# revdotcom/reverb

Measured on AMD Instinct MI355X. Metric: RTFx (audio-sec/wall-sec) Reverb-ASR attention_rescoring, higher is better.
Workload: dtype bf16

## Files before the change

### reverb_amd/_lib.py

```python
from __future__ import annotations

import ctypes as C
import os

_HERE = os.path.dirname(os.path.abspath(__file__))
LIB_PATH = os.path.join(_HERE, "librvb.so")

RVB_F32, RVB_BF16, RVB_FP8 = 0, 1, 2
ACT_NONE, ACT_SILU, ACT_RELU = 0, 1, 2
NORM_LN, NORM_AFFINE = 0, 1


class RvbError(RuntimeError):
    pass


class AudioInfo(C.Structure):
    _fields_ = [("container", C.c_int32), ("sample_format", C.c_int32), ("channels", C.c_int32), ("sample_rate", C.c_int32),
                ("bits_per_sample", C.c_int32), ("md5_checked", C.c_int32), ("frames", C.c_int64), ("decode_threads", C.c_int32),
                ("reserved", C.c_int32)]


class _SizedCfg(C.Structure):

# ... 104 lines not shown

class AttnTestArgs(C.Structure):
    _fields_ = ([(n, C.c_int32) for n in ("dtype", "heads", "dk", "nseq")] +
                [f for b in ("q", "k", "v", "out") for f in ((b, _f32p), (b[0] + "_rows", C.c_int32), (b[0] + "_stride", C.c_int32),
                                                             (b[0] + "_col", C.c_int32), ("pad_" + b, C.c_int32))] +
                [("p", _f32p), ("p_rows", C.c_int32), ("p_stride", C.c_int32), ("p_col", C.c_int32), ("p_off", C.c_int32),
                 ("bias_u", _f32p), ("bias_v", _f32p)] +
                [(n, _i32p) for n in ("q_start", "q_len", "kv_start", "kv_len", "q_pos0", "kv_index", "work")] +
                [(n, C.c_int32) for n in ("n_index", "n_work", "max_q", "q_block", "causal", "chunk", "left", "plain_order", "fold",
                                          "k_prefolded", "fold_kv_cap", "lab")] +
                [("ran", C.c_int32 * 8)])


class NormTestArgs(C.Structure):
    _fields_ = ([(n, C.c_int32) for n in ("dtype", "x_bf16", "mode", "silu", "out_f32", "out_fp8", "out2_fp8", "M", "d", "pad0")] +
                [(n, C.c_float) for n in ("eps", "eps2", "out_scale", "out2_scale")] +
                [(n, _f32p) for n in ("x", "gamma", "beta", "add", "gamma2", "beta2", "out", "out2")] +
                [("sat", C.c_uint32), ("sat2", C.c_uint32)])


_u32p = C.POINTER(C.c_uint32)

TEST_SIGNATURES = {
    "rvb_test_rownorm_ex": (C.c_int, [C.POINTER(NormTestArgs)]),
    "rvb_test_conv1_ex": (C.c_int, [C.c_int, _f32p, _f32p, _f32p, _f32p, _f32p, _f32p, C.c_int, C.c_int, C.c_int, C.c_int, C.c_float,
                                    _f32p, _u32p]),
    "rvb_test_embed": (C.c_int, [_f32p, C.c_int, _f32p, C.c_int, _i32p, _i32p, _f32p, C.c_int, C.c_int, C.c_float]),
    "rvb_test_amax_abs": (C.c_int, [C.c_int, _f32p, C.c_int64, _f32p]),
    "rvb_test_convert_f32": (C.c_int, [C.c_int, _f32p, _f32p, C.c_int64]),
    "rvb_test_gather_cache": (C.c_int, [C.c_void_p, C.c_void_p, _i32p, C.c_int, C.c_int, C.c_int, C.c_int]),
    "rvb_test_gather_pairs": (C.c_int, [_f32p, C.c_int, C.c_int64, _i32p, _i32p, C.c_int, _f32p]),
    "rvb_test_gemm": (C.c_int, [C.c_int, _f32p, _f32p, _f32p, _f32p, _f32p, C.c_int, C.c_int, C.c_int, C.c_float,
                                C.c_int, C.c_int, C.c_int, C.c_int, C.c_int, C.c_int, C.c_int]),
    "rvb_test_rownorm": (C.c_int, [C.c_int, _f32p, _f32p, _f32p, C.c_float, C.c_int, C.c_int, _f32p, _f32p, C.c_int,
                                   C.c_int, C.c_int]),
    "rvb_test_conv_block32": (C.c_int, [_f32p, _f32p, _f32p, _f32p, _f32p, _f32p, C.c_int, C.c_int, C.c_int]),
    "rvb_test_conv_s2sc": (C.c_int, [_f32p, _f32p, _f32p, _f32p, _f32p, _f32p, _f32p, C.c_int, C.c_int, C.c_int]),
    "rvb_test_conv1": (C.c_int, [C.c_int, _f32p, _f32p, _f32p, _f32p, _f32p, _f32p, C.c_int, C.c_int, C.c_int, C.c_int]),
    "rvb_test_conv_igemm_fp8": (C.c_int, [_f32p, _f32p, _f32p, _f32p, _f32p, _f32p, C.c_int, C.c_int, C.c_int, C.c_int, C.c_int, C.c_int, C.c_int,
                                           C.c_float, C.c_float, _f32p, _f32p, _f32p]),
    "rvb_test_joint_new": (C.c_void_p, [C.c_int, C.c_int, C.c_int, C.c_int, C.c_double, C.c_double, C.c_double]),
    "rvb_test_joint_free": (None, [C.c_void_p]),
    "rvb_test_joint_begin": (C.c_int, [C.c_void_p, C.c_int, _f32p, _i32p, C.c_int, C.c_float, C.c_float, _i32p, _i32p, _i32p, _i32p, _i32p,
                                       C.c_int]),
    "rvb_test_joint_finish": (C.c_int, [C.c_void_p, _f32p]),
    "rvb_test_joint_prefix": (C.c_int, [C.c_void_p, C.c_int, _i32p, _i32p]),
    "rvb_test_joint_result": (C.c_int, [C.c_void_p, _i32p, _i32p, _i32p, _f64p, _i32p, _f64p]),
    "rvb_test_glu_dwconv": (C.c_int, [C.c_int, _f32p, _f32p, _f32p, _f32p, _i32p, _f32p, C.c_int, C.c_int, C.c_int,
                                      C.c_int, C.c_int, _f32p, C.c_int]),
    "rvb_test_attention": (C.c_int, [C.c_int, _f32p, _f32p, _f32p, _f32p, _f32p, _f32p, _f32p, C.c_int, C.c_int,
                                     C.c_int, C.c_int, C.c_int, _i32p, _i32p, _i32p, _i32p, C.c_int, C.c_int]),
    "rvb_test_attention_trie": (C.c_int, [C.c_int, _f32p, _f32p, _f32p, _f32p, C.c_int, C.c_int, C.c_int, _i32p, _i32p, _i32p,
                                          _i32p, _i32p, _i32p, C.c_int, C.c_int, C.c_int]),
    "rvb_test_attention_ex": (C.c_int, [C.POINTER(AttnTestArgs)]),
    "rvb_test_attention_pos_bias": (C.c_int, [_f32p, C.c_int, C.c_int, C.c_int, C.c_int, _f32p, _f32p, C.c_int, C.c_int, C.c_float, _f32p]),
    "rvb_test_logsoftmax_topk": (C.c_int, [_f32p, C.c_int, C.c_int, C.c_int, C.c_float, C.c_int, _f32p, _i32p, _f32p]),
    "rvb_test_lse_gather": (C.c_int, [_f32p, C.c_int, C.c_int, _i32p, _f32p]),
    "rvb_test_ctc_viterbi": (C.c_int, [_f32p, C.c_int, C.c_int, _i32p, C.c_int, C.c_int, C.c_int, _i32p, _f32p]),
    "rvb_test_ctc_viterbi_wild": (C.c_int, [_f32p, C.c_int, C.c_int, _f32p, C.c_float, _i32p, C.c_int, C.c_int, C.c_int, _i32p, _f32p]),
    "rvb_test_ctc_viterbi_graph": (C.c_int, [_f32p, _i32p, C.c_int, C.c_int, _f32p, C.c_float, _i32p, _i32p, _i32p, _i32p, _u8p, C.c_int,
                                             C.c_int, _i32p, _i32p, _f32p]),
    "rvb_test_ctc_score": (C.c_int, [_f32p, C.c_int, C.c_int, _i32p, C.c_int, C.c_int, C.c_int, _f64p, _f32p, _f32p, _f32p, _i32p]),
    "rvb_test_ctc_score_batch": (C.c_int, [_f32p, _i32p, C.c_int, _i32p, _i32p, C.c_int, C.c_int, C.c_int, _f64p, _f32p, _f32p, _f32p,
                                           _i32p]),
    "rvb_test_ctc_find": (C.c_int, [_f32p, _i32p, C.c_int, C.c_int, _f32p, _i32p, _i32p, C.c_int, _f32p, C.c_int, C.c_int, C.c_int, C.c_int,
                                    _i64p, _i32p, _i32p, _f32p, _i32p, _i32p, _i32p, _f32p]),
    "rvb_test_gemm_glu": (C.c_int, [_f32p, _f32p, _f32p, _f32p, C.c_int, C.c_int, C.c_int]),
    "rvb_test_gemm_rowadd": (C.c_int, [_f32p, _f32p, _f32p, _f32p, _f32p, C.c_int, C.c_int, C.c_int, C.c_int, C.c_int, C.c_int]),
    "rvb_test_mp3_decode": (C.c_int64, [C.c_char_p, C.c_int64, C.c_int, _f32p, C.c_int64, _i64p, _i64p, C.c_int]),
    "rvb_test_mp3_hybrid": (C.c_int, [_f32p, _f32p, C.c_int, C.c_int, _f32p]),
    "rvb_test_mp3_polyphase": (C.c_int, [_f32p, _f32p, _i32p, _f32p]),
    "rvb_test_mp3_window": (C.c_int, [_f32p]),
    "rvb_test_mp3_huffman": (C.c_int, [C.c_int, C.POINTER(C.c_uint16), C.POINTER(C.c_uint8), _i32p]),
    "rvb_test_gemm_fp8": (C.c_int, [_f32p, _f32p, _f32p, _f32p, _f32p, C.c_int, C.c_int, C.c_int, C.c_float, C.c_float, C.c_int, C.c_int,
                                    C.c_float, _f32p, _f32p]),
    "rvb_test_rownorm_fp8": (C.c_int, [_f32p, _f32p, _f32p, C.c_float, C.c_int, C.c_int, C.c_int, C.c_float, _f32p, _f32p, _f32p,
                                       C.c_float, C.c_float, _f32p, _f32p]),
    "rvb_test_lse_gather_multi": (C.c_int, [_f32p, C.c_int, C.c_int, _i32p, _i32p, C.c_int, _f32p]),
    "rvb_test_row_xent": (C.c_int, [_f32p, C.c_int, C.c_int, C.c_int, _i32p, _i32p, _f32p, _f32p, _f64p, _i32p]),
    "rvb_test_host_pool": (C.c_int, [C.c_int, C.c_int, C.c_int]),
    "rvb_test_build_trie": (C.c_int, [_i32p, _i32p, _i32p, C.c_int, C.c_int, C.c_int, C.c_int, C.c_int, _i32p, _i32p, _i32p, _i32p, _i32p, _i32p,
                                      _i32p, _i32p, _i32p, _i32p, _i32p]),
    "rvb_test_fbank": (C.c_int, [_i16p, C.c_int64, _f32p]),
    "rvb_test_set_gemm_variant": (C.c_int, [C.c_int]),
    "rvb_test_set_gemm2_opts": (C.c_int, [C.c_int, C.c_int]),
    "rvb_test_gemm_timeline": (C.c_int, [C.c_int] * 6 + [C.POINTER(C.c_longlong), C.c_int, _i32p]),
    "rvb_test_gemm_bench": (C.c_int, [C.c_int, C.c_int, C.c_int, C.c_int, C.c_int, C.c_int, C.c_int, C.c_int, C.c_int,
                                      _f64p, _f64p]),
    "rvb_test_prefix_beam": (C.c_int, [_f32p, _i32p, C.c_int, C.c_int, C.c_int, _i32p, _i32p, _i32p, _i32p, _i32p,
                                       _f64p]),
    "rvb_test_prefix_beam_context": (C.c_int, [_f32p, _i32p, C.c_int, C.c_int, C.c_int, C.c_int, _i32p, _i32p, C.c_int, C.c_double,
                                               _i32p, _i32p, _i32p, _i32p, _i32p, _f64p, _f64p]),
    "rvb_test_context_walk": (C.c_int, [_i32p, _i32p, C.c_int, C.c_double, C.c_int, C.c_int, _i32p, C.c_int, _i32p, _f64p, _i32p,
                                        _f64p]),
    "rvb_test_window_stats": (C.c_int, [_f32p, C.c_int64, C.c_int64, C.c_int, C.c_int64, C.c_int, C.c_float, _f32p]),
    "rvb_test_sinc_conv": (C.c_int, [C.c_int, _f32p, C.c_int64, _f32p, C.c_int, C.c_int, C.c_int, C.c_int64, _f32p]),
    "rvb_test_pool_norm": (C.c_int, [C.c_int, C.c_int, _f32p, C.c_int, C.c_int, C.c_int, C.c_int, C.c_int, _f32p, _f32p, C.c_float,
                                     C.c_int, _f32p, C.c_int64, C.c_int64, C.c_int, _f32p, _f32p, C.c_float, C.c_float, _f32p]),
    "rvb_test_conv1d5": (C.c_int, [C.c_int, _f32p, C.c_int64, _f32p, _f32p, _f32p, C.c_int64]),
    "rvb_test_lstm_layer": (C.c_int, [C.c_int, _f32p, C.c_int, C.c_int, C.c_int, _f32p, _f32p, _f32p, _f32p, _f32p]),
    "rvb_test_classifier": (C.c_int, [C.c_int, _f32p, C.c_int, _f32p, _f32p, _f32p, C.POINTER(C.c_uint8), C.c_int64, C.c_int, C.c_int]),
    "rvb_test_tstp": (C.c_int, [C.c_int, _f32p, C.c_int, _i32p, _f32p, C.c_int, C.c_int, C.c_int, C.c_int, C.c_int, _f32p]),
    "rvb_test_conv2d": (C.c_int, [C.c_int, C.c_int, _f32p, _f32p, _f32p, _f32p, _f32p, C.c_int, C.c_int, C.c_int, C.c_int, C.c_int,
                                  C.c_int, C.c_int, C.c_int, _f32p, _f32p, C.c_int, C.c_int, C.c_int, C.c_int, _i32p]),
    "rvb_test_emb_stem": (C.c_int, [C.c_int, _f32p, C.c_int64, _i64p, C.c_int, C.c_int, C.c_int, C.c_int, C.c_int, C.c_int, _f32p, _f32p,
                                    _f32p, _f32p]),
}



class DiarCfg(_SizedCfg):
    _fields_ = [(n, C.c_int32) for n in (
        "struct_size", "dtype", "sample_rate", "window_samples", "step_samples", "sinc_filters", "sinc_channels", "lstm_hidden",
        "lstm_layers", "linear_dim", "linear_layers", "num_classes", "emb_channels", "emb_dim")]


DIAR_SIGNATURES = {
    "rvd_last_error": (C.c_char_p, []),
    "rvd_model_cfg_size": (C.c_int, []),
    "rvd_emb_windows_per_pass": (C.c_int, [_eng]),
    "rvd_create": (C.c_int, [C.POINTER(DiarCfg), C.c_int, C.POINTER(_eng)]),
    "rvd_destroy": (None, [_eng]),
    "rvd_load_tensor": (C.c_int, [_eng, C.c_char_p, _f32p, _i64p, C.c_int]),
    "rvd_finalize": (C.c_int, [_eng]),
    "rvd_num_windows": (C.c_int64, [_eng, C.c_int64]),
    "rvd_frames_per_window": (C.c_int, [_eng]),
    "rvd_upload_pcm": (C.c_int, [_eng, _i16p, C.c_int64]),
    "rvd_rerun_resident": (C.c_int, [_eng]),
    "rvd_resample_pcm": (C.c_int, [_eng, _i16p, C.c_int64, C.c_int, _i16p, _i64p]),
    "rvd_segment": (C.c_int, [_eng, C.c_int64, C.c_int, _f32p]),
    "rvd_get_classes": (C.c_int, [_eng, C.POINTER(C.c_uint8)]),
    "rvd_get_tap": (C.c_int, [_eng, C.c_char_p, _f32p]),
    "rvd_embed": (C.c_int, [_eng, _i64p, _f32p, C.c_int, _f32p]),
    "rvd_get_emb_fbank": (C.c_int, [_eng, C.c_int64, _f32p, _i32p]),
    "rvd_centroid_linkage": (C.c_int, [_eng, _f64p, C.c_int, C.c_int, _f64p]),
    "rvd_set_linkage_workgroups": (C.c_int, [_eng, C.c_int]),
    "rvd_get_emb_fp8": (C.c_int, [_eng, _i32p, _f32p, _i32p, C.POINTER(C.c_uint32)]),
    "rvd_set_emb_fp8_scales": (C.c_int, [_eng, _f32p, C.c_int32]),
    "rvd_set_profiling": (C.c_int, [_eng, C.c_int]),
    "rvd_reset_timings": (C.c_int, [_eng]),
    "rvd_get_timing": (C.c_int, [_eng, C.c_char_p, _f64p, _f64p, _i64p]),
}

_lib = None
_test_lib = None
TEST_LIB_PATH = os.path.join(_HERE, "librvb_test.so")


def load_test():
    global _test_lib
    if _test_lib is not None:
        return _test_lib
    if not os.path.exists(TEST_LIB_PATH):
        raise RvbError(f"{TEST_LIB_PATH} not found: run `python -m reverb_amd.build` (hipcc, gfx950)")
    lib = C.CDLL(TEST_LIB_PATH)
    for name, (res, args) in list(SIGNATURES.items()) + list(DIAR_SIGNATURES.items()) + list(TEST_SIGNATURES.items()):
        fn = getattr(lib, name)
        fn.restype = res
        fn.argtypes = args
    _test_lib = lib
    return lib


def load():
    global _lib
    if os.environ.get("RVB_LAB") == "1":
# ... 49 lines not shown
```

### reverb_amd/csrc/diar_engine.hip

```cpp
#include <cmath>
#include <cstdlib>
#include <cstring>
#include <map>
#include <string>
#include <vector>

#include "../../include/rvd.h"
#include "engine.h"

using namespace rvb;

#define RVD_TRY(expr) do { int _r = (expr); if (_r != OK) return _r; } while (0)

namespace {
struct LstmLayer { Linear ih; DevBuf whh; int in_pad = 0; };
constexpr int SINC_K = 251, SINC_STRIDE = 10, CONV_K = 5;
struct ConvW { DevBuf w, b, w_ig; int cin = 0, cout = 0, taps = 9, stride = 1;
               DevBuf w_ig_sc, b_sc;
               DevBuf w8, w8s; };
struct ResBlock { ConvW c1, c2, sc; bool has_sc = false; };
constexpr int FB_WIN = 400, FB_SHIFT = 160, FB_MEL = 80;
static int emb_batch() {
  static int v = [] { const char* e = getenv("RVD_EMB_BATCH"); const int x = e ? atoi(e) : 0; return x > 0 ? x : 768; }();
  return v;
}
#define EMB_BATCH (e->emb_batch > 0 ? e->emb_batch : (e->emb_batch = emb_batch()))
}

struct rvd_engine {
  rvd_model_cfg cfg;
  int device = 0, dtype = 0;
  int linkage_workgroups = 0;
  hipStream_t stream = nullptr;
  bool finalized = false;
  std::map<std::string, HostTensor> host;

  int f1 = 0, p1 = 0, f2 = 0, p2 = 0, f3 = 0, p3 = 0, cpad = 0;

  DevBuf filt, fsum;
  float wn_gamma = 1.f, wn_beta = 0.f;
  LNorm norm[3];
  Linear conv2, conv3;
  std::vector<LstmLayer> lstm;
  std::vector<Linear> lin;
  DevBuf cls_w, cls_b;
  DevBuf stage;

  DevBuf pcm, wave, craw;
  int64_t n_samples = 0, n_pad = 0, n_windows = 0, craw_frames = 0;

  DevBuf stats, a1, c2, a2, c3, a3, xproj, hA, hB, l0, l1, logp, cls;
  int last_W = 0;
  const void* last_lstm = nullptr;

  bool has_emb = false;
  DevBuf stem_w, stem_b;
  std::vector<std::vector<ResBlock>> stages;
  Linear seg1;
  DevBuf fb_window, fb_twiddle, fb_melw, fb_lo, fb_hi;
  DevBuf pcm_pad, emb_fb;
  int64_t emb_frames = 0;
  int nfr = 0;
  DevBuf act[4][4];
  int emb_batch = 0;
  bool emb_fp8 = false, want_fp8 = false;
  int emb_f8_state = 0;
  DevBuf act8[4][3], d_amax8, d_sat8;
  std::vector<float> scale8;
  int act_cap = 0;
  DevBuf e_win, e_mean, e_item_b, e_mask, e_stats, e_out;

  bool profiling = false;
  std::map<std::string, ProfEntry> prof;
  struct Pending { hipEvent_t a, b; std::string name; };
  std::vector<Pending> pending;
  std::vector<hipEvent_t> event_pool;
};

namespace {

struct DScope {
  rvd_engine* e; hipEvent_t a = nullptr, b = nullptr; std::string name;
  DScope(rvd_engine* e_, const char* n, double flops = 0.0) : e(e_), name(n) {
    auto& pe = e->prof[name];
    pe.launches += 1; pe.flops += flops;
    if (!e->profiling) return;
    auto get = [&]() { hipEvent_t ev; if (!e->event_pool.empty()) { ev = e->event_pool.back(); e->event_pool.pop_back(); } else (void)hipEventCreate(&ev); return ev; };
    a = get(); b = get();
    (void)hipEventRecord(a, e->stream);
  }
  ~DScope() { if (a) { (void)hipEventRecord(b, e->stream); e->pending.push_back({a, b, name}); } }
};
void drain(rvd_engine* e) {
  if (e->pending.empty()) return;
  (void)hipStreamSynchronize(e->stream);
  for (auto& p : e->pending) {
    float ms = 0.f;
    (void)hipEventElapsedTime(&ms, p.a, p.b);
    e->prof[p.name].ms += ms;
    e->event_pool.push_back(p.a); e->event_pool.push_back(p.b);
  }
  e->pending.clear();
}

int up_f32(rvd_engine* e, DevBuf& dst, const float* src, size_t n) {
  RVD_TRY(dst.ensure(n * 4));
  RVB_HIP_CHECK(hipMemcpyAsync(dst.p, src, n * 4, hipMemcpyHostToDevice, e->stream));
  RVB_HIP_CHECK(hipStreamSynchronize(e->stream));
  return OK;
}
int pack_T(rvd_engine* e, DevBuf& dst, const float* src, size_t n) {
  RVD_TRY(dst.ensure(n * dt_size(e->dtype)));
  if (e->dtype == DT_F32) return up_f32(e, dst, src, n);
  RVD_TRY(up_f32(e, e->stage, src, n));
  RVD_TRY(convert_f32(e->stream, e->dtype, e->stage.as<float>(), dst.p, n));
  RVB_HIP_CHECK(hipStreamSynchronize(e->stream));
  return OK;
}
int need(rvd_engine* e, const std::string& name, size_t numel, const HostTensor** out) {
  auto it = e->host.find(name);
  if (it == e->host.end()) { set_error("missing tensor: " + name); return E_STATE; }
  if (it->second.numel() != numel) {
    set_error("tensor " + name + " has " + std::to_string(it->second.numel()) + " elements, expected " + std::to_string(numel));
    return E_ARG;
  }
  *out = &it->second;
  return OK;
}
int pack_norm(rvd_engine* e, LNorm& n, const std::string& p, int d) {
  const HostTensor *g, *b;
  RVD_TRY(need(e, p + ".weight", d, &g));
  RVD_TRY(need(e, p + ".bias", d, &b));
  n.eps = 1e-5f;
  RVD_TRY(up_f32(e, n.g, g->data.data(), d));
  return up_f32(e, n.b, b->data.data(), d);
}

void sinc_filters(const float* low_hz_, const float* band_hz_, int npair, int sr, std::vector<float>* out, std::vector<float>* fsum) {
  const int K = SINC_K, half = K / 2;
  out->assign((size_t)2 * npair * K, 0.f);
  fsum->assign((size_t)2 * npair, 0.f);
  const double min_low = 50.0, min_band = 50.0;
// ... 137 lines not shown
  RVD_TRY(e->c2.ensure((size_t)R1 * CP * ts));
  RVD_TRY(e->a2.ensure((size_t)(R2 + 8) * CP * ts));
  RVD_TRY(e->c3.ensure((size_t)R2 * CP * ts));
  RVD_TRY(e->a3.ensure((size_t)R3 * CP * ts));
  RVD_TRY(e->xproj.ensure((size_t)R3 * 8 * H * ts));
  RVD_TRY(e->hA.ensure((size_t)R3 * 2 * H * ts));
  RVD_TRY(e->hB.ensure((size_t)R3 * 2 * H * ts));
  RVD_TRY(e->l0.ensure((size_t)R3 * c.linear_dim * ts));
  RVD_TRY(e->l1.ensure((size_t)R3 * c.linear_dim * ts));
  RVD_TRY(e->logp.ensure((size_t)R3 * c.num_classes * 4));
  RVD_TRY(e->cls.ensure((size_t)R3));

  { DScope sc(e, "window_stats");
    RVD_TRY(window_stats(e->stream, e->wave.as<float>(), first, W, c.step_samples, c.window_samples, 1e-5f, e->stats.as<float>())); }
  PoolNormArgs pn{};
  pn.W = W; pn.eps = 1e-5f;
  { DScope sc(e, "pool_norm");
    pn.x = nullptr; pn.frames_in = e->f1; pn.C = NF; pn.ld_out = NF;
    pn.gamma = e->norm[0].g.as<float>(); pn.beta = e->norm[0].b.as<float>(); pn.out = e->a1.p;
    pn.craw = e->craw.p; pn.craw_frame0 = first * (c.step_samples / SINC_STRIDE);
    pn.craw_frames_per_step = c.step_samples / SINC_STRIDE;
    pn.stats = e->stats.as<float>(); pn.fsum = e->fsum.as<float>(); pn.wn_gamma = e->wn_gamma; pn.wn_beta = e->wn_beta;
    RVD_TRY(pool_norm(e->stream, e->dtype, pn)); }
  RVD_TRY(run_sincnet_conv(e, e->a1.p, NF, e->conv2, e->c2.p, CP, R1));
  { DScope sc(e, "pool_norm");
    pn.x = e->c2.p; pn.rows_in = e->p1; pn.ld_in = CP; pn.frames_in = e->f2; pn.C = c.sinc_channels; pn.ld_out = CP;
    pn.gamma = e->norm[1].g.as<float>(); pn.beta = e->norm[1].b.as<float>(); pn.out = e->a2.p;
    RVD_TRY(pool_norm(e->stream, e->dtype, pn)); }
  RVD_TRY(run_sincnet_conv(e, e->a2.p, CP, e->conv3, e->c3.p, CP, R2));
  { DScope sc(e, "pool_norm");
    pn.x = e->c3.p; pn.rows_in = e->p2; pn.ld_in = CP; pn.frames_in = e->f3; pn.C = c.sinc_channels; pn.ld_out = CP;
    pn.gamma = e->norm[2].g.as<float>(); pn.beta = e->norm[2].b.as<float>(); pn.out = e->a3.p;
    RVD_TRY(pool_norm(e->stream, e->dtype, pn)); }

  const void* x = e->a3.p;
  int ldx = CP;
  for (int l = 0; l < c.lstm_layers; ++l) {
    RVD_TRY(run_gemm(e, "lstm_inproj", x, ldx, e->lstm[l].ih, e->xproj.p, 8 * H, R3, ACT_NONE));
    void* out = (l & 1) ? e->hB.p : e->hA.p;
    { DScope sc(e, "lstm_recurrence", 2.0 * (double)R3 * 8 * H * H);
      RVD_TRY(lstm_recurrence(e->stream, e->dtype, e->xproj.p, e->lstm[l].whh.p, out, W, e->p3)); }
    x = out; ldx = 2 * H;
  }
  e->last_lstm = x;
  for (int i = 0; i < c.linear_layers; ++i) {
    void* out = (i & 1) ? e->l1.p : e->l0.p;
    RVD_TRY(run_gemm(e, "linear", x, ldx, e->lin[i], out, c.linear_dim, R3, ACT_LRELU));
    x = out; ldx = c.linear_dim;
  }
  { DScope sc(e, "classifier");
    RVD_TRY(classifier_logsoftmax(e->stream, e->dtype, x, ldx, e->cls_w.as<float>(), e->cls_b.as<float>(), e->logp.as<float>(),
                                  e->cls.as<uint8_t>(), R3, ldx, c.num_classes)); }
  e->last_W = W;
  if (logp_out) {
    DScope sc(e, "d2h");
    RVB_HIP_CHECK(hipMemcpyAsync(logp_out, e->logp.p, (size_t)R3 * c.num_classes * 4, hipMemcpyDeviceToHost, e->stream));
  }
  RVB_HIP_CHECK(hipStreamSynchronize(e->stream));
  return OK;
}

int make_hamming_fbank_tables(rvd_engine* e) {
  const int NFFT = 512, NBIN = 257;
  const double PI = 3.14159265358979323846;
  std::vector<float> win(FB_WIN), tw(2 * 256), melw((size_t)FB_MEL * NBIN, 0.f);
  std::vector<int32_t> lo(FB_MEL, NBIN), hi(FB_MEL, 0);
  for (int i = 0; i < FB_WIN; ++i) win[i] = (float)(0.54 - 0.46 * std::cos(2.0 * PI * i / (FB_WIN - 1)));
  for (int k = 0; k < 256; ++k) { tw[2 * k] = (float)std::cos(2.0 * PI * k / NFFT); tw[2 * k + 1] = (float)(-std::sin(2.0 * PI * k / NFFT)); }
  auto mel = [](double f) { return 1127.0 * std::log(1.0 + f / 700.0); };
  const double mlo = mel(20.0), mhi = mel(8000.0), delta = (mhi - mlo) / (FB_MEL + 1);
  for (int m = 0; m < FB_MEL; ++m) {
    const double left = mlo + m * delta, center = left + delta, right = center + delta;
    for (int b = 0; b < NFFT / 2; ++b) {
      const double mf = mel(16000.0 / NFFT * b);
      const double w = std::max(0.0, std::min((mf - left) / (center - left), (right - mf) / (right - center)));
      if (w > 0.0) { melw[(size_t)m * NBIN + b] = (float)w; lo[m] = std::min(lo[m], b); hi[m] = std::max(hi[m], b + 1); }
    }
    if (hi[m] == 0) lo[m] = 0;
  }
  RVD_TRY(up_f32(e, e->fb_window, win.data(), win.size()));
  RVD_TRY(up_f32(e, e->fb_twiddle, tw.data(), tw.size()));
  RVD_TRY(up_f32(e, e->fb_melw, melw.data(), melw.size()));
  RVD_TRY(up_f32(e, e->fb_lo, (const float*)lo.data(), lo.size()));
  return up_f32(e, e->fb_hi, (const float*)hi.data(), hi.size());
}

int pack_conv_bn(rvd_engine* e, ConvW& c, const std::string& conv, const std::string& bn, int cout, int cin, int k, int stride) {
  const HostTensor *w, *g, *b, *m, *v;
  RVD_TRY(need(e, conv + ".weight", (size_t)cout * cin * k * k, &w));
  RVD_TRY(need(e, bn + ".weight", cout, &g));
  RVD_TRY(need(e, bn + ".bias", cout, &b));
  RVD_TRY(need(e, bn + ".running_mean", cout, &m));
  RVD_TRY(need(e, bn + ".running_var", cout, &v));
  const int CK = 64 / (int)dt_size(e->dtype);
  if (cin % CK) { set_error("embedding conv " + conv + ": input channels must be a multiple of " + std::to_string(CK)); return E_UNSUPPORTED; }
  const int taps = k * k;
  std::vector<float> pw((size_t)taps * cin * cout), pb(cout), sc(cout);
  for (int o = 0; o < cout; ++o) {
    sc[o] = g->data[o] / std::sqrt(v->data[o] + 1e-5f);
    pb[o] = b->data[o] - m->data[o] * sc[o];
  }
  conv_pack_direct(w->data.data(), sc.data(), cout, cin, taps, CK, pw.data());
  c.cin = cin; c.cout = cout; c.taps = taps; c.stride = stride;
  RVD_TRY(pack_T(e, c.w, pw.data(), pw.size()));
  if (conv_igemm_packed(e->dtype, k, stride, cin, cout)) {
    std::vector<float> pg((size_t)cout * taps * cin);
    conv_pack_igemm(w->data.data(), sc.data(), cout, cin, taps, (size_t)taps * cin, pg.data());
    RVD_TRY(pack_T(e, c.w_ig, pg.data(), pg.size()));
    if (e->emb_fp8 && cin % 128 == 0) {
      std::vector<uint8_t> q(pg.size());
      std::vector<float> ws(cout);
      const size_t K = (size_t)taps * cin;
      for (int o = 0; o < cout; ++o) {
        float am = 0.f;
        for (size_t kk = 0; kk < K; ++kk) am = std::max(am, std::fabs(pg[(size_t)o * K + kk]));
        ws[o] = am > 0.f ? am / 448.f : 1.f;
        const float inv = 1.f / ws[o];
        for (size_t kk = 0; kk < K; ++kk) q[(size_t)o * K + kk] = f32_to_fp8_host(pg[(size_t)o * K + kk] * inv);
      }
      RVD_TRY(c.w8.ensure(q.size()));
      RVB_HIP_CHECK(hipMemcpyAsync(c.w8.p, q.data(), q.size(), hipMemcpyHostToDevice, e->stream));
      RVD_TRY(up_f32(e, c.w8s, ws.data(), ws.size()));
      RVB_HIP_CHECK(hipStreamSynchronize(e->stream));
    }
  }
  return up_f32(e, c.b, pb.data(), pb.size());
}

int pack_fused_shortcut(rvd_engine* e, ResBlock& B, const std::string& p) {
  const char* f = lab_env("RVD_CONV_SC_FUSE");
  if ((f && atoi(f) == 0) || !B.has_sc || !B.c2.w_ig.p || B.sc.cin % 64 || B.sc.taps != 1) return OK;
  const int cout = B.c2.cout, cin = B.c2.cin, c2 = B.sc.cin;
  const HostTensor *w, *g, *b, *m, *v, *ws, *gs, *bs, *ms, *vs;
  RVD_TRY(need(e, p + ".conv2.weight", (size_t)cout * cin * 9, &w));
  RVD_TRY(need(e, p + ".bn2.weight", cout, &g));
  RVD_TRY(need(e, p + ".bn2.bias", cout, &b));
  RVD_TRY(need(e, p + ".bn2.running_mean", cout, &m));
  RVD_TRY(need(e, p + ".bn2.running_var", cout, &v));
  RVD_TRY(need(e, p + ".shortcut.0.weight", (size_t)cout * c2, &ws));
  RVD_TRY(need(e, p + ".shortcut.1.weight", cout, &gs));
  RVD_TRY(need(e, p + ".shortcut.1.bias", cout, &bs));
  RVD_TRY(need(e, p + ".shortcut.1.running_mean", cout, &ms));
  RVD_TRY(need(e, p + ".shortcut.1.running_var", cout, &vs));
  std::vector<float> pg((size_t)cout * (9 * (size_t)cin + c2)), pb(cout), sc(cout), ss(cout);
  for (int o = 0; o < cout; ++o) {
    sc[o] = g->data[o] / std::sqrt(v->data[o] + 1e-5f);
    ss[o] = gs->data[o] / std::sqrt(vs->data[o] + 1e-5f);
    pb[o] = (b->data[o] - m->data[o] * sc[o]) + (bs->data[o] - ms->data[o] * ss[o]);
  }
  conv_pack_fused_shortcut(w->data.data(), sc.data(), ws->data.data(), ss.data(), cout, cin, c2, pg.data());
  RVD_TRY(pack_T(e, B.c2.w_ig_sc, pg.data(), pg.size()));
  return up_f32(e, B.c2.b_sc, pb.data(), pb.size());
}

int finalize_embedding(rvd_engine* e) {
  const rvd_model_cfg& c = e->cfg;
  const std::string S = "embedding.resnet.";
  const int m = c.emb_channels;
  if (m != 32) { set_error("embedding: this build supports m_channels = 32 (ResNet34 of pyannote/wespeaker-voxceleb-resnet34-LM)"); return E_UNSUPPORTED; }
  { const char* f8 = lab_env("RVD_EMB_FP8"); e->emb_fp8 = (e->want_fp8 || (f8 && atoi(f8) == 1)) && e->dtype == DT_BF16; e->emb_f8_state = 0; }
  const HostTensor *w, *g, *b, *mu, *v;
  RVD_TRY(need(e, S + "conv1.weight", (size_t)m * 9, &w));
  RVD_TRY(need(e, S + "bn1.weight", m, &g));
  RVD_TRY(need(e, S + "bn1.bias", m, &b));
  RVD_TRY(need(e, S + "bn1.running_mean", m, &mu));
  RVD_TRY(need(e, S + "bn1.running_var", m, &v));
  std::vector<float> sw((size_t)m * 9), sb(m);
// ... 261 lines not shown
      g.A = e->e_stats.p; g.W = e->seg1.w.p; g.bias = e->seg1.b.as<float>(); g.C = e->e_out.p;
      g.M = ni; g.N = c.emb_dim; g.K = stats; g.lda = stats; g.ldw = stats; g.ldc = c.emb_dim; g.alpha = 1.f; g.act = ACT_NONE;
      g.out_f32 = 1;
      RVD_TRY(gemm(e->stream, e->dtype, g)); }
    RVB_HIP_CHECK(hipMemcpyAsync(emb_out + (size_t)i0 * c.emb_dim, e->e_out.p, (size_t)ni * c.emb_dim * 4, hipMemcpyDeviceToHost, e->stream));
    RVB_HIP_CHECK(hipStreamSynchronize(e->stream));
    i0 = i1;
  }
  return OK;
}

int fetch_T(rvd_engine* e, const void* src, int64_t rows, int ld, int cols, float* out) {
  const size_t ts = dt_size(e->dtype);
  std::vector<char> tmp((size_t)rows * ld * ts);
  RVB_HIP_CHECK(hipMemcpy(tmp.data(), src, tmp.size(), hipMemcpyDeviceToHost));
  for (int64_t r = 0; r < rows; ++r)
    for (int cc = 0; cc < cols; ++cc)
      out[r * cols + cc] = e->dtype == DT_BF16 ? bf16_to_f32(((const bf16_t*)tmp.data())[r * ld + cc]) : ((const float*)tmp.data())[r * ld + cc];
  return OK;
}

}

extern "C" {

const char* rvd_last_error(void) { return rvb::last_error(); }

int rvd_model_cfg_size(void) { return (int)sizeof(rvd_model_cfg); }

int rvd_emb_windows_per_pass(rvd_engine* e) {
  if (!e) { set_error("rvd_emb_windows_per_pass: null engine"); return E_ARG; }
  return EMB_BATCH;
}

int rvd_create(const rvd_model_cfg* cfg, int device, rvd_engine** out) {
  if (!cfg || !out) { set_error("rvd_create: null argument"); return E_ARG; }
  *out = nullptr;
  if (cfg->struct_size != (int32_t)sizeof(rvd_model_cfg)) {
    set_error("rvd_create: ABI mismatch: rvd_model_cfg.struct_size is " + std::to_string(cfg->struct_size) + ", this library's struct has " +
              std::to_string(sizeof(rvd_model_cfg)) + " bytes (bind it field by field from include/rvd.h)");
    return E_ARG;
  }
  if (cfg->dtype != DT_F32 && cfg->dtype != DT_BF16 && cfg->dtype != RVB_FP8) { set_error("rvd_create: dtype must be RVB_F32, RVB_BF16 or RVB_FP8"); return E_ARG; }
  if (cfg->lstm_hidden != 128 || cfg->sinc_filters != 80 || cfg->sinc_filters % 8 || cfg->sinc_channels < 1 || cfg->sinc_channels > 64 ||
      cfg->lstm_layers < 1 || cfg->linear_layers < 0 || cfg->linear_layers > 2 || (cfg->linear_layers && cfg->linear_dim % 8) ||
      cfg->linear_dim > 256 || cfg->num_classes < 1 || cfg->num_classes > 16 || cfg->sample_rate != 16000 ||
      cfg->step_samples % (SINC_STRIDE * 4) || cfg->step_samples <= 0 || cfg->window_samples < 4000) {
    set_error("rvd_create: unsupported model dimensions (this build: 80 sinc filters, <= 64 conv channels, LSTM hidden 128, 16 kHz)");
    return E_ARG;
  }
  int ndev = 0;
  if (hipGetDeviceCount(&ndev) != hipSuccess || ndev <= device || device < 0) {
    set_error("rvd_create: no HIP device " + std::to_string(device) + " (this library has no CPU fallback)");
    return E_HIP;
  }
  RVB_HIP_CHECK(hipSetDevice(device));
  rvd_engine* e = new rvd_engine();
  e->cfg = *cfg; e->device = device;
  e->want_fp8 = cfg->dtype == RVB_FP8;
  e->dtype = e->want_fp8 ? (int)DT_BF16 : cfg->dtype;
  e->cfg.dtype = e->dtype;
  RVB_HIP_CHECK(hipStreamCreateWithFlags(&e->stream, hipStreamNonBlocking));
  e->f1 = (cfg->window_samples - SINC_K) / SINC_STRIDE + 1; e->p1 = e->f1 / 3;
  e->f2 = e->p1 - (CONV_K - 1); e->p2 = e->f2 / 3;
  e->f3 = e->p2 - (CONV_K - 1); e->p3 = e->f3 / 3;
  e->cpad = 64;
  *out = e;
  return OK;
}

void rvd_destroy(rvd_engine* e) {
  if (!e) return;
  (void)hipSetDevice(e->device);
  (void)hipStreamSynchronize(e->stream);
  drain(e);
  for (auto ev : e->event_pool) (void)hipEventDestroy(ev);
  DevBuf* bufs[] = {&e->filt, &e->fsum, &e->cls_w, &e->cls_b, &e->stage, &e->pcm, &e->wave, &e->craw, &e->stats, &e->a1, &e->c2,
                    &e->a2, &e->c3, &e->a3, &e->xproj, &e->hA, &e->hB, &e->l0, &e->l1, &e->logp, &e->cls, &e->conv2.w, &e->conv2.b,
                    &e->conv3.w, &e->conv3.b};
  for (auto* b : bufs) b->release();
  for (auto& n : e->norm) { n.g.release(); n.b.release(); }
  for (auto& l : e->lstm) { l.ih.w.release(); l.ih.b.release(); l.whh.release(); }
  for (auto& l : e->lin) { l.w.release(); l.b.release(); }
  DevBuf* ebufs[] = {&e->stem_w, &e->stem_b, &e->seg1.w, &e->seg1.b, &e->fb_window, &e->fb_twiddle, &e->fb_melw, &e->fb_lo, &e->fb_hi,
                     &e->pcm_pad, &e->emb_fb, &e->e_win, &e->e_mean, &e->e_item_b, &e->e_mask, &e->e_stats, &e->e_out};
  for (auto* b : ebufs) b->release();
  for (auto& st : e->stages)
    for (auto& blk : st)
      for (ConvW* cw : {&blk.c1, &blk.c2, &blk.sc}) { cw->w.release(); cw->b.release(); cw->w_ig.release(); cw->w_ig_sc.release(); cw->b_sc.release(); cw->w8.release(); cw->w8s.release(); }
  for (auto& row : e->act) for (auto& b : row) b.release();
  (void)hipStreamDestroy(e->stream);
  delete e;
}

int rvd_load_tensor(rvd_engine* e, const char* name, const float* host, const int64_t* shape, int ndim) {
  if (!e || !name || !host || ndim < 0 || (ndim && !shape)) { set_error("rvd_load_tensor: null argument"); return E_ARG; }
  if (e->finalized) { set_error("rvd_load_tensor: engine already finalized"); return E_STATE; }
  HostTensor t;
  t.shape.assign(shape, shape + ndim);
  t.data.assign(host, host + t.numel());
  e->host[name] = std::move(t);
  return OK;
}

int rvd_finalize(rvd_engine* e) {
  if (!e) { set_error("rvd_finalize: null engine"); return E_ARG; }
  if (e->finalized) { set_error("rvd_finalize: already finalized"); return E_STATE; }
  RVB_HIP_CHECK(hipSetDevice(e->device));
  return finalize_impl(e);
}

int64_t rvd_num_windows(const rvd_engine* e, int64_t n) {
  if (!e || n <= 0) return 0;
  const int64_t win = e->cfg.window_samples, step = e->cfg.step_samples;
  const int64_t full = n >= win ? (n - win) / step + 1 : 0;
  const bool tail = n < win || (n - win) % step > 0;
  return full + (tail ? 1 : 0);
}
int rvd_frames_per_window(const rvd_engine* e) { return e ? e->p3 : 0; }

static int prepare_audio(rvd_engine* e, int64_t n);

int rvd_upload_pcm(rvd_engine* e, const int16_t* pcm, int64_t n) {
  if (!e || !pcm || n <= 0) { set_error("rvd_upload_pcm: null or empty audio"); return E_ARG; }
  if (!e->finalized) { set_error("rvd_upload_pcm: finalize the model first"); return E_STATE; }
  RVB_HIP_CHECK(hipSetDevice(e->device));
  RVD_TRY(e->pcm.ensure((size_t)n * 2));
  { DScope sc(e, "h2d");
    RVB_HIP_CHECK(hipMemcpyAsync(e->pcm.p, pcm, (size_t)n * 2, hipMemcpyHostToDevice, e->stream)); }
  return prepare_audio(e, n);
}

int rvd_rerun_resident(rvd_engine* e) {
  if (!e) { set_error("rvd_rerun_resident: null engine"); return E_ARG; }
  if (e->n_samples <= 0 || !e->pcm.p) { set_error("rvd_rerun_resident: upload audio first"); return E_STATE; }
  RVB_HIP_CHECK(hipSetDevice(e->device));
  return prepare_audio(e, e->n_samples);
}

int rvd_resample_pcm(rvd_engine* e, const int16_t* pcm, int64_t n, int sample_rate, int16_t* out, int64_t* n_out) {
  if (!e || !pcm || n <= 0 || !n_out) { set_error("rvd_resample_pcm: null or empty audio"); return E_ARG; }
  if (sample_rate < 1000 || sample_rate > 384000) { set_error("rvd_resample_pcm: sample rate out of range"); return E_ARG; }
  const int target = e->cfg.sample_rate;
  std::vector<float> ker;
  int orig, nw, width, K;
  resample_taps(sample_rate, target, &ker, &orig, &nw, &width, &K);
  const int64_t m = ((int64_t)nw * n + orig - 1) / orig;
  if (!out) { *n_out = m; return OK; }
  if (*n_out < m) { set_error("rvd_resample_pcm: output buffer too small"); return E_ARG; }
  *n_out = m;
  RVB_HIP_CHECK(hipSetDevice(e->device));
  DevBuf src, taps, res, dst;
  int r = src.ensure((size_t)n * 2 + 16);
  if (r == OK) r = taps.ensure(ker.size() * 4);
  if (r == OK) r = res.ensure((size_t)m * 4);
  if (r == OK) r = dst.ensure((size_t)m * 2);
  if (r == OK && hipMemcpyAsync(src.p, pcm, (size_t)n * 2, hipMemcpyHostToDevice, e->stream) != hipSuccess) r = E_HIP;
  if (r == OK && hipMemcpyAsync(taps.p, ker.data(), ker.size() * 4, hipMemcpyHostToDevice, e->stream) != hipSuccess) r = E_HIP;
  if (r == OK) { DScope sc(e, "resample"); r = resample(e->stream, src.as<int16_t>(), n, taps.as<float>(), orig, nw, width, K, res.as<float>(), m); }
  if (r == OK) r = round_to_i16(e->stream, res.as<float>(), m, dst.as<int16_t>());
  if (r == OK && hipMemcpyAsync(out, dst.p, (size_t)m * 2, hipMemcpyDeviceToHost, e->stream) != hipSuccess) r = E_HIP;
  if (hipStreamSynchronize(e->stream) != hipSuccess && r == OK) r = E_HIP;
  src.release(); taps.release(); res.release(); dst.release();
  if (r == E_HIP) set_error("rvd_resample_pcm: device copy or kernel failed");
  return r;
}

static int prepare_audio(rvd_engine* e, int64_t n) {
  const rvd_model_cfg& c = e->cfg;
  e->n_samples = n;
  e->n_windows = rvd_num_windows(e, n);
  e->n_pad = (e->n_windows - 1) * c.step_samples + c.window_samples;
  e->craw_frames = (e->n_pad - SINC_K) / SINC_STRIDE + 1;
  RVD_TRY(e->wave.ensure((size_t)e->n_pad * 4));
  RVD_TRY(e->craw.ensure((size_t)e->craw_frames * c.sinc_filters * dt_size(e->dtype)));
  { DScope sc(e, "pcm_to_float");
    RVD_TRY(pcm_to_float(e->stream, e->pcm.as<int16_t>(), n, e->wave.as<float>(), e->n_pad)); }
  { DScope sc(e, "sinc_conv", 2.0 * (double)e->craw_frames * c.sinc_filters * SINC_K);
    RVD_TRY(sinc_conv(e->stream, e->dtype, e->wave.as<float>(), e->filt.as<float>(), e->craw.p, e->craw_frames, c.sinc_filters,
                      SINC_K, SINC_STRIDE)); }
  if (e->has_emb) {
    e->emb_frames = (e->n_pad - FB_WIN) / FB_SHIFT + 1;
    RVD_TRY(e->pcm_pad.ensure((size_t)e->n_pad * 2));
    RVD_TRY(e->emb_fb.ensure((size_t)e->emb_frames * FB_MEL * 4));
    RVB_HIP_CHECK(hipMemsetAsync(e->pcm_pad.p, 0, (size_t)e->n_pad * 2, e->stream));
    RVB_HIP_CHECK(hipMemcpyAsync(e->pcm_pad.p, e->pcm.p, (size_t)n * 2, hipMemcpyDeviceToDevice, e->stream));
    DScope sc(e, "emb_fbank");
    FbankTables t{e->fb_window.as<float>(), e->fb_twiddle.as<float>(), e->fb_melw.as<float>(), e->fb_lo.as<int>(), e->fb_hi.as<int>()};
    RVD_TRY(fbank(e->stream, e->pcm_pad.as<int16_t>(), e->emb_frames, e->emb_fb.as<float>(), t));
    RVD_TRY(e->e_mean.ensure((size_t)e->n_windows * FB_MEL * 4));
    RVD_TRY(emb_window_mean(e->stream, e->emb_fb.as<float>(), nullptr, (int)e->n_windows, c.step_samples / FB_SHIFT, e->nfr, e->e_mean.as<float>()));
  }
  RVB_HIP_CHECK(hipStreamSynchronize(e->stream));
  return OK;
}

int rvd_segment(rvd_engine* e, int64_t first_window, int n_windows, float* logp_out) {
  if (!e) { set_error("rvd_segment: null engine"); return E_ARG; }
  RVB_HIP_CHECK(hipSetDevice(e->device));
  return segment_impl(e, first_window, n_windows, logp_out);
}

int rvd_get_classes(rvd_engine* e, uint8_t* out) {
  if (!e || !out) { set_error("rvd_get_classes: null argument"); return E_ARG; }
  if (e->last_W <= 0) { set_error("rvd_get_classes: no rvd_segment call yet"); return E_STATE; }
  RVB_HIP_CHECK(hipSetDevice(e->device));
  RVB_HIP_CHECK(hipMemcpy(out, e->cls.p, (size_t)e->last_W * e->p3, hipMemcpyDeviceToHost));
  return OK;
}

int rvd_get_tap(rvd_engine* e, const char* name, float* out) {
  if (!e || !name || !out) { set_error("rvd_get_tap: null argument"); return E_ARG; }
  if (e->last_W <= 0) { set_error("rvd_get_tap: no rvd_segment call yet"); return E_STATE; }
  RVB_HIP_CHECK(hipSetDevice(e->device));
  const int64_t R3 = (int64_t)e->last_W * e->p3;
  if (!strcmp(name, "sincnet")) return fetch_T(e, e->a3.p, R3, e->cpad, e->cfg.sinc_channels, out);
  if (!strcmp(name, "lstm")) return fetch_T(e, e->last_lstm, R3, 2 * e->cfg.lstm_hidden, 2 * e->cfg.lstm_hidden, out);
  set_error(std::string("rvd_get_tap: unknown tap ") + name);
  return E_ARG;
}

int rvd_embed(rvd_engine* e, const int64_t* win, const float* mask, int n, float* emb_out) {
  if (!e || !win || !mask || !emb_out || n < 0) { set_error("rvd_embed: null argument"); return E_ARG; }
  RVB_HIP_CHECK(hipSetDevice(e->device));
  return embed_impl(e, win, mask, n, emb_out);
}
int rvd_get_emb_fbank(rvd_engine* e, int64_t window, float* out, int32_t* n_frames) {
  if (!e || !out) { set_error("rvd_get_emb_fbank: null argument"); return E_ARG; }
  if (!e->has_emb || e->n_windows == 0) { set_error("rvd_get_emb_fbank: needs an embedding model and uploaded audio"); return E_STATE; }
  if (window < 0 || window >= e->n_windows) { set_error("rvd_get_emb_fbank: window outside the uploaded audio"); return E_ARG; }
  RVB_HIP_CHECK(hipSetDevice(e->device));
  const int64_t f0 = window * (e->cfg.step_samples / FB_SHIFT);
  RVB_HIP_CHECK(hipMemcpy(out, e->emb_fb.as<float>() + f0 * FB_MEL, (size_t)e->nfr * FB_MEL * 4, hipMemcpyDeviceToHost));
  if (n_frames) *n_frames = e->nfr;
  return OK;
}

int rvd_centroid_linkage(rvd_engine* e, const double* X, int n, int d, double* Z) {
  if (!e || !X || !Z || n < 1 || d < 1) { set_error("rvd_centroid_linkage: bad argument"); return E_ARG; }
  if (n > 46000) { set_error("rvd_centroid_linkage: more than 46000 points"); return E_UNSUPPORTED; }
  if (n == 1) return OK;
  RVB_HIP_CHECK(hipSetDevice(e->device));
  DevBuf dX, dD, dI, dM, dZ, dC;
  int rc = OK;
  do {
    if ((rc = dC.ensure(4096)) != OK) break;
    if ((rc = dX.ensure((size_t)n * d * 8)) != OK) break;
    if ((rc = dD.ensure((size_t)n * n * 8)) != OK) break;
    if ((rc = dI.ensure((size_t)3 * n * 4)) != OK) break;
    if ((rc = dM.ensure((size_t)n * 8)) != OK) break;
    if ((rc = dZ.ensure((size_t)(n - 1) * 4 * 8)) != OK) break;
    std::vector<int> init((size_t)3 * n);
    for (int i = 0; i < n; ++i) { init[i] = i; init[n + i] = -1; ((uint16_t*)&init[2 * (size_t)n])[i] = 1; }
    std::vector<double> inf(n, INFINITY);
    (void)hipMemcpyAsync(dX.p, X, (size_t)n * d * 8, hipMemcpyHostToDevice, e->stream);
    (void)hipMemcpyAsync(dI.p, init.data(), init.size() * 4, hipMemcpyHostToDevice, e->stream);
    (void)hipMemcpyAsync(dM.p, inf.data(), (size_t)n * 8, hipMemcpyHostToDevice, e->stream);
    (void)hipStreamSynchronize(e->stream);
    {
      DScope sc(e, "linkage");
      rc = centroid_linkage(e->stream, dX.as<double>(), n, d, dD.as<double>(), (uint16_t*)(dI.as<int>() + 2 * n), dI.as<int>(),
                            dI.as<int>() + n, dM.as<double>(), dZ.as<double>(), dC.p, e->linkage_workgroups);
    }
    if (rc != OK) break;
    if (hipMemcpyAsync(Z, dZ.p, (size_t)(n - 1) * 4 * 8, hipMemcpyDeviceToHost, e->stream) != hipSuccess ||
        hipStreamSynchronize(e->stream) != hipSuccess) {
      set_error(std::string("rvd_centroid_linkage: ") + hipGetErrorString(hipGetLastError()));
      rc = E_HIP;
      break;
    }
    { double retries = 0.0;
// ... 74 lines not shown
```

### reverb_amd/csrc/engine.h

```cpp
#pragma once
#include <condition_variable>
#include <functional>
#include <map>
#include <memory>
#include <mutex>
#include <string>
#include <thread>
#include <vector>

#include "../../include/rvb.h"
#include "kernels.h"
#include "search.h"

namespace rvb {

struct HostTensor {
  std::vector<float> data;
  std::vector<int64_t> shape;
  size_t numel() const { size_t n = 1; for (auto s : shape) n *= (size_t)s; return n; }
};

struct DevBuf {
  void* p = nullptr;
  size_t bytes = 0;
// ... 120 lines not shown
           int V, int blank_id, bool allow_wild = false);
  int begin(hipStream_t s);
  bool touches(int r0, int nrows) const;
  int advance(hipStream_t s, const float* lp, int ld, int r0, int nrows, const float* wmax = nullptr, float bias = 0.f);
  int finish(hipStream_t s, int32_t* states , float* score );
  void release();
};

struct CtcGraphAligner {
  std::vector<GraphSeq> seq;
  std::vector<int32_t> h_tokens, h_arc_off, h_finals, h_rows;
  std::vector<uint32_t> h_arcs;
  int max_N = 0, blank = 0;
  bool has_wild = false;
  size_t alpha_floats = 0, bp_bytes = 0;
  int64_t total_frames = 0;
  DevBuf d_tokens, d_arc_off, d_arcs, d_finals, d_rows, d_seqs, d_alpha, d_bp, d_states, d_score;
  int plan(const char* who, const int32_t* node_tokens, const int32_t* n_nodes, const int32_t* pred_off, const int32_t* preds,
           const uint8_t* is_final, int n_seq, const std::vector<std::vector<int32_t>>& seq_rows, int V, int blank_id);
  int begin(hipStream_t s);
  bool touches(int r0, int nrows) const;
  int advance(hipStream_t s, const float* lp, int ld, int r0, int nrows, const float* wmax = nullptr, float bias = 0.f);
  int finish(hipStream_t s, int32_t* states , float* score );
  void release();
};

struct CtcScorer {
  CtcAligner lat;
  bool post = false;
  DevBuf d_csum, d_loglik, d_llhat, d_coff, d_arows, d_beta, d_z, d_acc;
  int plan(const char* who, const int32_t* tokens, const int32_t* tok_lens, int n_seq, const std::vector<std::vector<int32_t>>& seq_rows,
           int V, int blank_id);
  int begin(hipStream_t s, bool posteriors);
  int advance(hipStream_t s, const float* lp, int ld, int r0, int nrows);
  int finish_forward(hipStream_t s, double* loglik );
  int advance_backward(hipStream_t s, const float* lp, int ld, int r0, int nrows);
  int finish_backward(hipStream_t s, float* occupancy, float* mean_frame, float* peak_post, int32_t* peak_frame );
  void release();
};


struct CtcFinder {
  std::vector<FindSeq> seq;
  std::vector<FindPhrase> phr;
  std::vector<int32_t> h_tokens, h_rows;
  int blank = 0, max_cand = 0;
  DevBuf d_tokens, d_rows, d_seqs, d_phr, d_h, d_st, d_count, d_cend, d_cstart, d_cscore;
  int plan(const char* who, const int32_t* tokens, const int32_t* tok_lens, int n_phrases, const float* threshold,
           const std::vector<std::vector<int32_t>>& seq_rows, int V, int blank_id, int max_candidates);
  int begin(hipStream_t s);
  bool touches(int r0, int nrows) const;
  int advance(hipStream_t s, const float* lp, int ld, int r0, int nrows, const float* wmax);
  int finish(hipStream_t s, int max_hits, int32_t* n_hits, int32_t* start, int32_t* end, float* score, int64_t* n_candidates,
             int32_t* raw_end = nullptr, int32_t* raw_start = nullptr, float* raw_score = nullptr);
  void release();
};

}

struct rvb_engine {
  rvb_model_cfg cfg;
  int device = 0;
  int dtype = 0;
  bool fp8 = false;
  int f8_state = 0;
  std::vector<rvb::F8Scales> f8;
  std::vector<unsigned> f8_groups;
  rvb::DevBuf d_amax;
  bool f8_conv2 = false;
  float f8_x1 = 0.f;
  rvb::DevBuf d_f8sat;
  hipStream_t stream = nullptr;
  bool finalized = false;

  std::map<std::string, rvb::HostTensor> host;

  rvb::DevBuf cmvn_mean, cmvn_istd, conv1_w, conv1_b;
  rvb::Linear conv2, embed_out, ctc;
  rvb::LNorm enc_after;
  std::vector<rvb::EncLayer> enc;
  rvb::Decoder dec_l, dec_r;
  rvb::DevBuf pe_f32;
  int pe_rows = 0;
  rvb::DevBuf fb_window, fb_twiddle, fb_melw, fb_lo, fb_hi;
  rvb::DevBuf stage;

  rvb::DevBuf pcm, feats;
  rvb::DevBuf pcm_next;
  hipStream_t copy_stream = nullptr;
  hipEvent_t pcm_ready = nullptr, pcm_free = nullptr;
  bool pcm_pending = false;
  int64_t n_samples_next = 0;
  rvb::DevBuf wave_f32, rs_kernel;
  rvb::DevBuf wave_in;
  bool pcm_is_float = false;
  int dec_chunk = 0, dec_left = -1;
  int64_t n_samples = 0, n_frames = 0, feat_rows = 0;

  int B = 0, T0 = 0, T1 = 0, F1 = 0, T2 = 0, F2 = 0, beam = 0;
  std::vector<int32_t> in_lens, enc_lens;
  rvb::DevBuf d_feats_in, X1, X2, x, xn, y, h, ao, dconv, enc_out, logits, topv, topi;
  rvb::DevBuf d_enc_lens, d_seq_start, d_seq_len, d_aux_i32;
  float* h_topv = nullptr;
  int32_t* h_topi = nullptr;
  size_t h_top_cap = 0;
  struct Slice { int c0, nb; hipEvent_t ev; bool done; };
  std::vector<Slice> slices;
  std::vector<hipEvent_t> slice_event_pool;
  int xattn_max_rows = 0;
  const int* cur_lens = nullptr;
  std::vector<rvb::PrefixResult> nbest;
  std::shared_ptr<const rvb::ContextGraph> context_graph;
  std::vector<rvb::RescoreResult> rescored;
  std::vector<rvb::TrieBatch> trie_l;
  rvb::HostPool pool;
  std::vector<rvb::JointResult> joint;
  std::vector<rvb::DevBuf> jkv;
  rvb::DevBuf jlogp, jpair_row, jpair_tok, jpair_out;
  int64_t joint_rows = 0, joint_steps = 0;
  float last_blank_penalty = 0.f;
  std::vector<std::vector<int>> attn_tokens;
  std::vector<float> attn_scores;
  rvb::DevBuf atopv, atopi;
  std::vector<rvb::DevBuf> kcache, vcache, kcache2, vcache2, memkv;
  rvb::DevBuf dx, dxn, dy, dh, dqkv, dq, dao, kvmem, d_tok, d_pos, d_tgt, d_logp;
  rvb::DevBuf d_hq_start, d_hq_len, d_hkv_start, d_hkv_len;
  rvb::DevBuf d_hq_pos0, d_hpath_start, d_hpath_len, d_path, d_work, d_tgt_ptr;
  int64_t rescore_rows = 0, rescore_pairs = 0;
  rvb::DevBuf d_xlse, d_xsum, d_xtop;

  struct StreamState {
    bool active = false;
    int offset = 0;
    int cache_len = 0;
    std::vector<rvb::DevBuf> kv, kv2;
    int cnn_rows = 0;
    std::vector<rvb::DevBuf> cnn, cnn2;
  } stream_st;
  rvb::DevBuf d_stream_i32;

  rvb::CtcAligner aligner;
  rvb::CtcScorer scorer;
  rvb::CtcFinder finder;
  rvb::CtcGraphAligner graph_aligner;
  rvb::DevBuf align_lp, align_tv, align_ti, align_row, align_col, align_out;

  void* comm = nullptr;
  int comm_world = 1, comm_rank = 0;
  rvb::DevBuf comm_send, comm_recv;

  int profiling = 0;
  std::map<std::string, rvb::ProfEntry> prof;
  struct Pending { hipEvent_t a, b; std::string name; };
  std::vector<Pending> pending;
  std::vector<hipEvent_t> event_pool;
};
```

### reverb_amd/csrc/engine.hip

```cpp
#include "engine.h"

#include <algorithm>
#include <atomic>
#include <condition_variable>
#include <functional>
#include <mutex>
#include <chrono>
#include <cmath>
#include <cstdlib>
#include <cstring>
#include <thread>

namespace rvb {

static thread_local std::string g_err;
void set_error(const std::string& msg) { g_err = msg; }
const char* last_error() { return g_err.c_str(); }

int DevBuf::ensure(size_t n) {
  if (n <= bytes && p) return OK;
  if (p) { (void)hipFree(p); p = nullptr; bytes = 0; }
  if (n == 0) n = 16;
  hipError_t err = hipMalloc(&p, n);
  if (err != hipSuccess) {
    p = nullptr;
    (void)hipGetLastError();
    set_error("hipMalloc of " + std::to_string(n) + " bytes failed: " + hipGetErrorString(err));
    return E_NOMEM;
  }
  bytes = n;
  return OK;
}
void DevBuf::release() { if (p) (void)hipFree(p); p = nullptr; bytes = 0; }

#define RVB_TRY(expr) do { int _r = (expr); if (_r != OK) return _r; } while (0)

struct Scope {
  rvb_engine* e; hipEvent_t a = nullptr, b = nullptr; std::string name;
  Scope(rvb_engine* e_, const char* n, double flops = 0.0, double bytes = 0.0) : e(e_), name(n) {
    auto& pe = e->prof[name];
    pe.launches += 1; pe.flops += flops; pe.bytes += bytes;
    if (e->profiling == 0 || (e->profiling == 2 && name != "gemm" && name != "gemm_fp8")) return;
    auto get = [&]() { hipEvent_t ev; if (!e->event_pool.empty()) { ev = e->event_pool.back(); e->event_pool.pop_back(); } else (void)hipEventCreate(&ev); return ev; };
    a = get(); b = get();
    (void)hipEventRecord(a, e->stream);
  }
  ~Scope() {
    if (!a) return;
    (void)hipEventRecord(b, e->stream);
    e->pending.push_back({a, b, name});
  }
};
static void drain_prof(rvb_engine* e) {
  if (e->pending.empty()) return;
  (void)hipStreamSynchronize(e->stream);
  for (auto& p : e->pending) {
    float ms = 0.f;
    (void)hipEventElapsedTime(&ms, p.a, p.b);
    e->prof[p.name].ms += ms;
    e->event_pool.push_back(p.a); e->event_pool.push_back(p.b);
  }
  e->pending.clear();
}

static int upload_f32(rvb_engine* e, DevBuf& dst, const float* src, size_t n) {
  RVB_TRY(dst.ensure(n * 4));
  RVB_HIP_CHECK(hipMemcpyAsync(dst.p, src, n * 4, hipMemcpyHostToDevice, e->stream));
  return OK;
}
static int upload_i32(rvb_engine* e, DevBuf& dst, const int32_t* src, size_t n) {
  RVB_TRY(dst.ensure(n * 4 + 16));
  if (n) RVB_HIP_CHECK(hipMemcpyAsync(dst.p, src, n * 4, hipMemcpyHostToDevice, e->stream));
  return OK;
}
static int pack_T(rvb_engine* e, DevBuf& dst, const float* src, size_t n) {
  RVB_TRY(dst.ensure(n * dt_size(e->dtype)));
  if (e->dtype == DT_F32) {
    RVB_HIP_CHECK(hipMemcpyAsync(dst.p, src, n * 4, hipMemcpyHostToDevice, e->stream));
    return OK;
  }
  RVB_TRY(e->stage.ensure(n * 4));
  RVB_HIP_CHECK(hipMemcpyAsync(e->stage.p, src, n * 4, hipMemcpyHostToDevice, e->stream));
  return convert_f32(e->stream, e->dtype, e->stage.as<float>(), dst.p, n);
// ... 44 lines not shown
}
static int pack_norm(rvb_engine* e, LNorm& n, const std::string& p, int d, float eps) {
  const HostTensor *g, *b;
  RVB_TRY(need(e, p + ".weight", d, &g));
  RVB_TRY(need(e, p + ".bias", d, &b));
  n.eps = eps;
  RVB_TRY(upload_f32(e, n.g, g->data.data(), d));
  return upload_f32(e, n.b, b->data.data(), d);
}
static int pack_concat(rvb_engine* e, Linear& L, const std::vector<std::string>& names, int out_each, int in, bool f8 = false) {
  std::vector<float> w((size_t)names.size() * out_each * in), b((size_t)names.size() * out_each);
  for (size_t i = 0; i < names.size(); ++i) {
    const HostTensor *tw, *tb;
    RVB_TRY(need(e, names[i] + ".weight", (size_t)out_each * in, &tw));
    RVB_TRY(need(e, names[i] + ".bias", out_each, &tb));
    memcpy(w.data() + i * (size_t)out_each * in, tw->data.data(), (size_t)out_each * in * 4);
    memcpy(b.data() + i * (size_t)out_each, tb->data.data(), (size_t)out_each * 4);
  }
  int r = pack_linear(e, L, w.data(), b.data(), (int)names.size() * out_each, in, f8);
  if (r == OK) (void)hipStreamSynchronize(e->stream);
  return r;
}
static int pack_lsl(rvb_engine* e, Linear& L, const std::string& p, int d, const float* cat, int ncat) {
  std::vector<float> w((size_t)d * d, 0.f), b(d, 0.f);
  for (int i = 0; i < ncat; ++i) {
    const HostTensor *tw, *tb;
    const std::string n = p + ".language_layers." + std::to_string(i);
    RVB_TRY(need(e, n + ".weight", (size_t)d * d, &tw));
    RVB_TRY(need(e, n + ".bias", d, &tb));
    const float c = cat[i];
    if (i == 0) {
      for (size_t k = 0; k < w.size(); ++k) w[k] = c * tw->data[k];
      for (int k = 0; k < d; ++k) b[k] = c * tb->data[k];
    } else {
      for (size_t k = 0; k < w.size(); ++k) w[k] = w[k] + c * tw->data[k];
      for (int k = 0; k < d; ++k) b[k] = b[k] + c * tb->data[k];
    }
  }
  int r = pack_linear(e, L, w.data(), b.data(), d, d);
  if (r == OK) (void)hipStreamSynchronize(e->stream);
  return r;
}

static void make_pe(int rows, int d, std::vector<float>* pe) {
  pe->assign((size_t)rows * d, 0.f);
  const float c = (float)(-(std::log(10000.0) / (double)d));
  for (int i = 0; i < d; i += 2) {
    const float div = std::exp((float)i * c);
    for (int pos = 0; pos < rows; ++pos) {
      const float ang = (float)pos * div;
      (*pe)[(size_t)pos * d + i] = std::sin(ang);
      if (i + 1 < d) (*pe)[(size_t)pos * d + i + 1] = std::cos(ang);
    }
  }
}

static int make_fbank_tables(rvb_engine* e) {
  const int WIN = 400, NFFT = 512, NBIN = 257, NMEL = 80;
  const double PI = 3.14159265358979323846;
  std::vector<float> win(WIN), tw(2 * 256), melw((size_t)NMEL * NBIN, 0.f);
  std::vector<int32_t> lo(NMEL, NBIN), hi(NMEL, 0);
  for (int i = 0; i < WIN; ++i) win[i] = (float)std::pow(0.5 - 0.5 * std::cos(2.0 * PI * i / (WIN - 1)), 0.85);
  for (int k = 0; k < 256; ++k) { tw[2 * k] = (float)std::cos(2.0 * PI * k / NFFT); tw[2 * k + 1] = (float)(-std::sin(2.0 * PI * k / NFFT)); }
  auto mel = [](double f) { return 1127.0 * std::log(1.0 + f / 700.0); };
  const double mlo = mel(20.0), mhi = mel(8000.0), delta = (mhi - mlo) / (NMEL + 1);
  for (int m = 0; m < NMEL; ++m) {
    const double left = mlo + m * delta, center = left + delta, right = center + delta;
    for (int b = 0; b < NFFT / 2; ++b) {
      const double mf = mel(16000.0 / NFFT * b);
      const double up = (mf - left) / (center - left), down = (right - mf) / (right - center);
      const double w = std::max(0.0, std::min(up, down));
      if (w > 0.0) {
        melw[(size_t)m * NBIN + b] = (float)w;
        lo[m] = std::min(lo[m], b); hi[m] = std::max(hi[m], b + 1);
      }
    }
    if (hi[m] == 0) lo[m] = 0;
  }
  RVB_TRY(upload_f32(e, e->fb_window, win.data(), win.size()));
  RVB_TRY(upload_f32(e, e->fb_twiddle, tw.data(), tw.size()));
  RVB_TRY(upload_f32(e, e->fb_melw, melw.data(), melw.size()));
  RVB_TRY(upload_i32(e, e->fb_lo, lo.data(), lo.size()));
  RVB_TRY(upload_i32(e, e->fb_hi, hi.data(), hi.size()));
  RVB_HIP_CHECK(hipStreamSynchronize(e->stream));
  return OK;
}

static int out_frames(int T0) { const int T1 = (T0 - 3) / 2 + 1; return (T1 - 3) / 2 + 1; }

static const AttnArgs& with_lab(AttnArgs& a) { attention_lab_switches(a); return a; }

static int reset_f8sat(rvb_engine* e) {
  static const int on = lab_env("RVB_FP8_SAT") ? atoi(lab_env("RVB_FP8_SAT")) : 1;
  if (!on) return OK;
  RVB_TRY(e->d_f8sat.ensure((e->enc.size() + 1) * 8 * 4));
  RVB_HIP_CHECK(hipMemsetAsync(e->d_f8sat.p, 0, (e->enc.size() + 1) * 8 * 4, e->stream));
  return OK;
}

static double gemm_alg_bytes(const rvb_engine* e, const GemmArgs& g) {
  const double es = g.in_fp8 ? 1.0 : (double)dt_size(e->dtype);
  const double a = g.conv ? (double)(g.M / (g.cT2 * g.cF2)) * g.cT1 * g.cF1 * g.cC * es : (double)g.M * g.K * es;
  const double c = (double)g.M * (g.act == ACT_GLU ? g.N / 2 : g.N) * (g.out_fp8 ? 1.0 : (g.out_f32 ? 4.0 : (double)dt_size(e->dtype)));
  return a + (double)g.N * g.K * es + (g.bias ? 4.0 * g.N : 0.0) + c + (g.res ? 4.0 * (double)g.M * g.N : 0.0);
}

static constexpr int GLU_FUSE_DEFAULT = 1;
static int run_gemm(rvb_engine* e, const void* A, int lda, const Linear& L, void* C, int ldc, int M, bool out_f32,
                    float alpha = 1.f, int act = ACT_NONE, const float* res = nullptr, int ldres = 0) {
  GemmArgs g;
  memset(&g, 0, sizeof(g));
  g.A = A; g.W = L.w.p; g.bias = L.b.as<float>(); g.res = res; g.C = C;
  g.M = M; g.N = L.out; g.K = L.in; g.lda = lda; g.ldw = L.in; g.ldc = ldc; g.ldres = ldres;
  g.alpha = alpha; g.act = act; g.out_f32 = out_f32 ? 1 : 0;
  Scope sc(e, "gemm", 2.0 * M * (double)L.out * L.in, gemm_alg_bytes(e, g));
  return gemm(e->stream, e->dtype, g);
}
static int run_norm(rvb_engine* e, const float* x, const LNorm& n, void* out, bool out_f32, int M, int d,
                    int mode = NORM_LN, int silu = 0, const void* add = nullptr, const LNorm* second = nullptr,
                    void* out2 = nullptr, float out8 = 0.f, float out2_8 = 0.f, bool x_bf16 = false, unsigned* sat = nullptr,
                    unsigned* sat2 = nullptr) {
  NormArgs a;
  a.sat = sat; a.sat2 = sat2;
  a.x_bf16 = x_bf16 ? 1 : 0;
  a.x = x; a.gamma = n.g.as<float>(); a.beta = n.b.as<float>(); a.eps = n.eps; a.mode = mode; a.silu = silu;
  a.add = add; a.out = out; a.out_f32 = out_f32 ? 1 : 0; a.M = M; a.d = d;
  if (second) { a.gamma2 = second->g.as<float>(); a.beta2 = second->b.as<float>(); a.eps2 = second->eps; a.out2 = out2; }
  if (out8 > 0.f) { a.out_fp8 = 1; a.out_inv_scale = 1.f / out8; }
  if (out2_8 > 0.f) { a.out2_fp8 = 1; a.out2_inv_scale = 1.f / out2_8; }
  Scope sc(e, "rownorm");
  return rownorm(e->stream, e->dtype, a);
}
static int run_gemm8(rvb_engine* e, const void* A8, int lda, const Linear& L, void* C, int ldc, int M, float a_scale, int out_kind,
                     float out_scale = 1.f, float alpha = 1.f, int act = ACT_NONE, const float* res = nullptr, int ldres = 0,
                     unsigned* sat = nullptr) {
  GemmArgs g;
  memset(&g, 0, sizeof(g));
  g.sat = sat;
  g.A = A8; g.W = L.w8.p; g.bias = L.b.as<float>(); g.res = res; g.C = C;
  g.M = M; g.N = L.out; g.K = L.in; g.lda = lda; g.ldw = L.in; g.ldc = ldc; g.ldres = ldres;
  g.alpha = alpha; g.act = act; g.out_f32 = out_kind == 1; g.out_fp8 = out_kind == 2; g.in_fp8 = 1;
  g.a_scale = a_scale; g.w_scale = L.wscale.as<float>(); g.out_inv_scale = 1.f / out_scale;
  if (!L.w8.p) { set_error("fp8 GEMM on a layer without fp8 weights"); return E_STATE; }
  Scope sc(e, "gemm_fp8", 2.0 * M * (double)L.out * L.in, gemm_alg_bytes(e, g));
  return gemm(e->stream, e->dtype, g);
}

static int pack_decoder(rvb_engine* e, Decoder& D, const std::string& p, int nblocks, const float* cat, int ncat) {
  const int d = e->cfg.d_model, V = e->cfg.vocab, ff = e->cfg.dec_ffn_dim;
  D.present = false;
  if (nblocks <= 0 || !find(e, p + ".embed.0.weight")) return OK;
  const HostTensor* emb;
  RVB_TRY(need(e, p + ".embed.0.weight", (size_t)V * d, &emb));
  RVB_TRY(upload_f32(e, D.embed, emb->data.data(), emb->data.size()));
  RVB_TRY(pack_norm(e, D.after, p + ".after_norm", d, 1e-5f));
  RVB_TRY(pack_named_linear(e, D.out, p + ".output_layer", V, d));
  D.layers.resize(nblocks);
  for (int j = 0; j < nblocks; ++j) {
    DecLayer& L = D.layers[j];
    const std::string q = p + ".decoders." + std::to_string(j);
    L.is_lsl = find(e, q + ".language_layers.0.weight") != nullptr;
    const float eps = L.is_lsl ? 1e-12f : 1e-5f;
    RVB_TRY(pack_concat(e, L.self_qkv, {q + ".self_attn.linear_q", q + ".self_attn.linear_k", q + ".self_attn.linear_v"}, d, d));
    RVB_TRY(pack_named_linear(e, L.self_out, q + ".self_attn.linear_out", d, d));
    RVB_TRY(pack_named_linear(e, L.src_q, q + ".src_attn.linear_q", d, d));
    RVB_TRY(pack_concat(e, L.src_kv, {q + ".src_attn.linear_k", q + ".src_attn.linear_v"}, d, d));
// ... 747 lines not shown
      t->path.push_back(node);
      asks.push_back({node, j < h.len ? seq(h, j) : eos});
    }
    const int n_own = t->R - first_new;
    t->hq_start.push_back(first_new); t->hq_len.push_back(n_own); t->hq_pos0.push_back(n_own ? own_pos0 : 0);
    t->hkv_len.push_back(h.len + 1);
    for (int q0 = 0; q0 < n_own; q0 += 16) { t->work.push_back((int32_t)t->hq_start.size() - 1); t->work.push_back(q0); }
  }
  if (cur_chunk >= 0) t->crow_len[cur_chunk] = t->R - t->crow_start[cur_chunk];
  for (int b = 0; b < B; ++b) t->max_chunk_rows = std::max(t->max_chunk_rows, t->crow_len[b]);
  t->P = (int)asks.size();
  t->tgt_ptr.assign(t->R + 1, 0);
  for (auto& a : asks) t->tgt_ptr[a.first + 1]++;
  for (int r = 0; r < t->R; ++r) t->tgt_ptr[r + 1] += t->tgt_ptr[r];
  std::vector<int32_t> fill(t->tgt_ptr.begin(), t->tgt_ptr.end() - 1);
  t->tgt.assign(t->P, 0); t->pair_slot.assign(t->P, 0);
  for (int p = 0; p < t->P; ++p) { const int slot = fill[asks[p].first]++; t->tgt[slot] = asks[p].second; t->pair_slot[p] = slot; }
}

static void build_chunk_trie(rvb_engine* e, int b, bool reversed, int sos, int eos, TrieBatch* t) {
  const PrefixResult& pr = e->nbest[b];
  std::vector<HypRef> hyps(pr.nbest.size());
  for (size_t i = 0; i < hyps.size(); ++i) hyps[i] = {b, (int)i, (int)pr.nbest[i].size(), 0};
  if (reversed)
    build_trie_range(hyps.data(), hyps.data() + hyps.size(), b, 1, sos, eos,
                     [&](const HypRef& h, int j) { return pr.nbest[h.idx][h.len - 1 - j]; }, t);
  else
    build_trie_range(hyps.data(), hyps.data() + hyps.size(), b, 1, sos, eos, [&](const HypRef& h, int j) { return pr.nbest[h.idx][j]; }, t);
}

static void merge_tries(const std::vector<TrieBatch>& part, TrieBatch* t) {
  const int B = (int)part.size();
  *t = TrieBatch();
  size_t nR = 0, nH = 0, nPath = 0, nP = 0, nW = 0;
  for (const TrieBatch& c : part) { nR += c.R; nH += c.hq_start.size(); nPath += c.path.size(); nP += c.P; nW += c.work.size(); }
  t->tok.reserve(nR); t->pos.reserve(nR); t->path.reserve(nPath); t->work.reserve(nW);
  t->hq_start.reserve(nH); t->hq_len.reserve(nH); t->hq_pos0.reserve(nH); t->hkv_start.reserve(nH); t->hkv_len.reserve(nH);
  t->tgt.reserve(nP); t->pair_slot.reserve(nP); t->tgt_ptr.reserve(nR + 1);
  t->crow_start.assign(B, 0); t->crow_len.assign(B, 0);
  for (int b = 0; b < B; ++b) {
    const TrieBatch& c = part[b];
    const int32_t R0 = t->R, H0 = (int32_t)t->hq_start.size(), PATH0 = (int32_t)t->path.size(), P0 = t->P;
    t->crow_start[b] = c.R ? R0 : 0; t->crow_len[b] = c.R;
    t->max_chunk_rows = std::max(t->max_chunk_rows, c.R);
    t->tok.insert(t->tok.end(), c.tok.begin(), c.tok.end());
    t->pos.insert(t->pos.end(), c.pos.begin(), c.pos.end());
    for (int32_t v : c.path) t->path.push_back(v + R0);
    for (int32_t v : c.hq_start) t->hq_start.push_back(v + R0);
    t->hq_len.insert(t->hq_len.end(), c.hq_len.begin(), c.hq_len.end());
    t->hq_pos0.insert(t->hq_pos0.end(), c.hq_pos0.begin(), c.hq_pos0.end());
    for (int32_t v : c.hkv_start) t->hkv_start.push_back(v + PATH0);
    t->hkv_len.insert(t->hkv_len.end(), c.hkv_len.begin(), c.hkv_len.end());
    for (size_t k = 0; k + 1 < c.work.size(); k += 2) { t->work.push_back(c.work[k] + H0); t->work.push_back(c.work[k + 1]); }
    for (int r = 0; r < c.R; ++r) t->tgt_ptr.push_back(c.tgt_ptr[r] + P0);
    t->tgt.insert(t->tgt.end(), c.tgt.begin(), c.tgt.end());
    for (int32_t v : c.pair_slot) t->pair_slot.push_back(v + P0);
    t->R += c.R; t->P += c.P;
  }
  t->tgt_ptr.push_back(t->P);
}

static void build_trie_parallel(rvb_engine* e, bool reversed, TrieBatch* t) {
  const int B = e->B, sos = e->cfg.sos_id, eos = e->cfg.eos_id;
  std::vector<TrieBatch> part(B);
  std::atomic<int> next(0);
  auto work = [&]() {
    for (int b = next.fetch_add(1); b < B; b = next.fetch_add(1)) build_chunk_trie(e, b, reversed, sos, eos, &part[b]);
  };
  e->pool.run(std::max(1u, std::min<unsigned>(search_threads(), (unsigned)B / 4)), work);
  merge_tries(part, t);
}

static int decoder_memory_kv(rvb_engine* e, Decoder& D, int M) {
  const int d = e->cfg.d_model;
  const size_t es = dt_size(e->dtype);
  for (auto& L : D.layers) {
    RVB_TRY(L.kvmem.ensure((size_t)M * 2 * d * es));
    RVB_TRY(run_gemm(e, e->enc_out.p, d, L.src_kv, L.kvmem.p, 2 * d, M, false));
  }
  D.kv_ready = true;
  return OK;
}

struct XentRows { std::vector<float> lse; std::vector<double> sum_x; std::vector<int32_t> top1; };
static int decoder_forward(rvb_engine* e, Decoder& D, const TrieBatch& t, std::vector<float>* logp, XentRows* xent = nullptr) {
  const rvb_model_cfg& c = e->cfg;
  const int d = c.d_model, heads = c.dec_heads, dk = d / heads, ff = c.dec_ffn_dim, V = c.vocab;
  const int M = e->B * e->T2, R = t.R, nhyp = (int)t.hq_start.size();
  const size_t es = dt_size(e->dtype);
  RVB_TRY(upload_i32(e, e->d_tok, t.tok.data(), R));
  RVB_TRY(upload_i32(e, e->d_pos, t.pos.data(), R));
  RVB_TRY(upload_i32(e, e->d_tgt, t.tgt.data(), t.P));
  RVB_TRY(upload_i32(e, e->d_tgt_ptr, t.tgt_ptr.data(), R + 1));
  RVB_TRY(upload_i32(e, e->d_path, t.path.data(), t.path.size()));
  RVB_TRY(upload_i32(e, e->d_work, t.work.data(), t.work.size()));
  RVB_TRY(upload_i32(e, e->d_hq_start, t.hq_start.data(), nhyp));
  RVB_TRY(upload_i32(e, e->d_hq_len, t.hq_len.data(), nhyp));
  RVB_TRY(upload_i32(e, e->d_hq_pos0, t.hq_pos0.data(), nhyp));
  RVB_TRY(upload_i32(e, e->d_hpath_start, t.hkv_start.data(), nhyp));
  RVB_TRY(upload_i32(e, e->d_hpath_len, t.hkv_len.data(), nhyp));
  RVB_TRY(upload_i32(e, e->d_hkv_start, t.crow_start.data(), e->B));
  RVB_TRY(upload_i32(e, e->d_hkv_len, t.crow_len.data(), e->B));
  RVB_TRY(e->dx.ensure((size_t)R * d * 4));
  RVB_TRY(e->dxn.ensure((size_t)R * d * es));
  RVB_TRY(e->dy.ensure((size_t)R * d * es));
  RVB_TRY(e->dao.ensure((size_t)R * d * es));
  RVB_TRY(e->dq.ensure((size_t)R * d * es));
  RVB_TRY(e->dqkv.ensure((size_t)R * 3 * d * es));
  RVB_TRY(e->dh.ensure((size_t)R * ff * es));
  if (!D.kv_ready) RVB_TRY(decoder_memory_kv(e, D, M));
  RVB_TRY(e->d_logp.ensure((size_t)t.P * 4));
  if (xent) {
    RVB_TRY(e->d_xlse.ensure((size_t)R * 4)); RVB_TRY(e->d_xsum.ensure((size_t)R * 8)); RVB_TRY(e->d_xtop.ensure((size_t)R * 4));
  }
  float* x = e->dx.as<float>();
  {
    Scope sc(e, "embed");
    RVB_TRY(embed_tokens(e->stream, D.embed.as<float>(), e->pe_f32.as<float>(), e->d_tok.as<int>(), e->d_pos.as<int>(),
                         x, R, d, std::sqrt((float)d)));
  }
  for (auto& L : D.layers) {
    RVB_TRY(run_norm(e, x, L.n1, e->dxn.p, false, R, d));
    RVB_TRY(run_gemm(e, e->dxn.p, d, L.self_qkv, e->dqkv.p, 3 * d, R, false));
    AttnArgs a;
    memset(&a, 0, sizeof(a));
    a.q = e->dqkv.p; a.k = (const char*)e->dqkv.p + (size_t)d * es; a.v = (const char*)e->dqkv.p + (size_t)2 * d * es;
    a.q_stride = a.k_stride = a.v_stride = 3 * d; a.o_stride = d; a.out = e->dao.p;
    a.q_start = e->d_hq_start.as<int>(); a.q_len = e->d_hq_len.as<int>(); a.q_pos0 = e->d_hq_pos0.as<int>();
    a.kv_start = e->d_hpath_start.as<int>(); a.kv_len = e->d_hpath_len.as<int>(); a.kv_index = e->d_path.as<int>();
    a.work = e->d_work.as<int>(); a.n_work = (int)t.work.size() / 2; a.q_block = 16;
    a.nseq = nhyp; a.heads = heads; a.dk = dk; a.max_q = 16; a.causal = 1; a.sqrt_dk = std::sqrt((float)dk);
    {
      Scope sc(e, "attention");
      RVB_TRY(attention(e->stream, e->dtype, with_lab(a)));
    }
    RVB_TRY(run_gemm(e, e->dao.p, d, L.self_out, x, d, R, true, 1.f, ACT_NONE, x, d));
    RVB_TRY(run_norm(e, x, L.n2, e->dxn.p, false, R, d));
    RVB_TRY(run_gemm(e, e->dxn.p, d, L.src_q, e->dq.p, d, R, false));
    memset(&a, 0, sizeof(a));
    a.q = e->dq.p; a.k = L.kvmem.p; a.v = (const char*)L.kvmem.p + (size_t)d * es;
    a.q_stride = d; a.k_stride = a.v_stride = 2 * d; a.o_stride = d; a.out = e->dao.p;
    a.q_start = e->d_hkv_start.as<int>(); a.q_len = e->d_hkv_len.as<int>();
    a.kv_start = e->d_aux_i32.as<int>(); a.kv_len = e->d_aux_i32.as<int>() + e->B;
    a.nseq = e->B; a.heads = heads; a.dk = dk; a.max_q = t.max_chunk_rows; a.causal = 0; a.sqrt_dk = std::sqrt((float)dk);
    {
      Scope sc(e, "attention");
      RVB_TRY(attention(e->stream, e->dtype, with_lab(a)));
    }
    RVB_TRY(run_gemm(e, e->dao.p, d, L.src_out, x, d, R, true, 1.f, ACT_NONE, x, d));
    RVB_TRY(run_norm(e, x, L.n3, e->dxn.p, false, R, d));
    const void* ffin = e->dxn.p;
    if (L.is_lsl) {
      RVB_TRY(run_gemm(e, e->dxn.p, d, L.lsl, e->dy.p, d, R, false));
      ffin = e->dy.p;
    }
    RVB_TRY(run_gemm(e, ffin, d, L.ff1, e->dh.p, ff, R, false, 1.f, ACT_RELU));
    RVB_TRY(run_gemm(e, e->dh.p, ff, L.ff2, x, d, R, true, 1.f, ACT_NONE, x, d));
  }
  RVB_TRY(run_norm(e, x, D.after, e->dxn.p, false, R, d));
  const int Vld = (V + 3) & ~3;
  for (int r0 = 0; r0 < R; r0 += LOGIT_SLAB) {
    const int rows = std::min(LOGIT_SLAB, R - r0);
    RVB_TRY(run_gemm(e, (const char*)e->dxn.p + (size_t)r0 * d * es, d, D.out, e->logits.p, Vld, rows, true));
    Scope sc(e, "lse_gather");
    if (xent)
      RVB_TRY(row_xent(e->stream, e->logits.as<float>(), rows, V, Vld, e->d_tgt_ptr.as<int>() + r0, e->d_tgt.as<int>(),
                       e->d_logp.as<float>(), e->d_xlse.as<float>() + r0, e->d_xsum.as<double>() + r0, e->d_xtop.as<int>() + r0));
    else
      RVB_TRY(lse_gather_multi(e->stream, e->logits.as<float>(), rows, V, Vld, e->d_tgt_ptr.as<int>() + r0, e->d_tgt.as<int>(),
                               e->d_logp.as<float>()));
  }
  logp->resize(t.P);
  RVB_HIP_CHECK(hipMemcpyAsync(logp->data(), e->d_logp.p, (size_t)t.P * 4, hipMemcpyDeviceToHost, e->stream));
  if (xent) {
    xent->lse.resize(R); xent->sum_x.resize(R); xent->top1.resize(R);
    RVB_HIP_CHECK(hipMemcpyAsync(xent->lse.data(), e->d_xlse.p, (size_t)R * 4, hipMemcpyDeviceToHost, e->stream));
    RVB_HIP_CHECK(hipMemcpyAsync(xent->sum_x.data(), e->d_xsum.p, (size_t)R * 8, hipMemcpyDeviceToHost, e->stream));
    RVB_HIP_CHECK(hipMemcpyAsync(xent->top1.data(), e->d_xtop.p, (size_t)R * 4, hipMemcpyDeviceToHost, e->stream));
  }
  RVB_HIP_CHECK(hipStreamSynchronize(e->stream));
  return OK;
}

static int rescore_impl(rvb_engine* e, double ctc_weight, double reverse_weight) {
  if ((int)e->nbest.size() != e->B || e->B <= 0) { set_error("rvb_attention_rescore before rvb_ctc_prefix_beam"); return E_STATE; }
  if (!e->dec_l.present) { set_error("model has no attention decoder"); return E_STATE; }
  RVB_TRY(wait_slices(e, -1));
  const bool use_r = reverse_weight > 0.0;
  if (use_r && !e->dec_r.present) { set_error("reverse_weight > 0 but model has no right-to-left decoder"); return E_STATE; }
  RVB_HIP_CHECK(hipSetDevice(e->device));
  const int B = e->B, T2 = e->T2, eos = e->cfg.eos_id, sos = e->cfg.sos_id;
  std::vector<HypRef> hyps;
  int P = 0;
  std::vector<int32_t> ckv(2 * (size_t)B);
  for (int b = 0; b < B; ++b) {
    const PrefixResult& pr = e->nbest[b];
    ckv[b] = b * T2; ckv[B + b] = e->enc_lens[b];
    for (size_t i = 0; i < pr.nbest.size(); ++i) {
      const int len = (int)pr.nbest[i].size();
      if (len + 1 > e->pe_rows) { set_error("hypothesis longer than the positional table"); return E_UNSUPPORTED; }
      hyps.push_back({b, (int)i, len, P});
      P += len + 1;
    }
  }
  RVB_TRY(upload_i32(e, e->d_aux_i32, ckv.data(), ckv.size()));
  TrieBatch tl, tr;
  const auto th0 = std::chrono::steady_clock::now();
  if ((int)e->trie_l.size() == B) merge_tries(e->trie_l, &tl);
  else build_trie_parallel(e, false, &tl);
  {
    auto& pe = e->prof["rescore_trie_host"];
    pe.ms += std::chrono::duration<double, std::milli>(std::chrono::steady_clock::now() - th0).count();
    pe.launches += 1;
  }
  std::vector<float> lslot, rslot;
  const auto td0 = std::chrono::steady_clock::now();
  RVB_TRY(decoder_forward(e, e->dec_l, tl, &lslot));
  {
    auto& pe = e->prof["rescore_decoder_wall"];
    pe.ms += std::chrono::duration<double, std::milli>(std::chrono::steady_clock::now() - td0).count();
    pe.launches += 1;
  }
  e->xattn_max_rows = tl.max_chunk_rows;
  e->rescore_rows = tl.R; e->rescore_pairs = tl.P;
  if (use_r) {
    build_trie_parallel(e, true, &tr);
    RVB_TRY(decoder_forward(e, e->dec_r, tr, &rslot));
    e->rescore_rows += tr.R; e->rescore_pairs += tr.P;
  }
  const auto ta0 = std::chrono::steady_clock::now();
  std::vector<float> logp(P), rlogp(use_r ? P : 0);
  for (int p = 0; p < P; ++p) { logp[p] = lslot[tl.pair_slot[p]]; if (use_r) rlogp[p] = rslot[tr.pair_slot[p]]; }

  e->rescored.assign(B, RescoreResult());
  std::vector<float> att_score(hyps.size());
  std::vector<int> best_hyp(B, -1);
  for (size_t hi = 0; hi < hyps.size(); ++hi) {
    const HypRef& hr = hyps[hi];
    const PrefixResult& pr = e->nbest[hr.chunk];
    RescoreResult& rr = e->rescored[hr.chunk];
    if (rr.logp.empty()) { rr.logp.resize(pr.nbest.size()); rr.rlogp.resize(pr.nbest.size()); rr.score = -INFINITY; }
    const float* lp = logp.data() + hr.row0;
    rr.logp[hr.idx].assign(lp, lp + hr.len + 1);
    float score = 0.f;
    for (int j = 0; j < hr.len; ++j) score += lp[j];
    score += lp[hr.len];
    if (use_r) {
      const float* rp = rlogp.data() + hr.row0;
      rr.rlogp[hr.idx].assign(rp, rp + hr.len + 1);
      float r_score = 0.f;
      for (int j = 0; j < hr.len; ++j) r_score += rp[hr.len - j - 1];
      r_score += rp[hr.len];
// ... 458 lines not shown
      return E_UNSUPPORTED;
    }
  RVB_HIP_CHECK(hipStreamSynchronize(e->stream));
  return OK;
}

}

using namespace rvb;

extern "C" {

const char* rvb_last_error(void) { return last_error(); }
const char* rvb_version(void) { return "librvb 0.1 (gfx950)"; }

}
namespace rvb {
#ifdef RVB_TEST_API
const char* lab_env(const char* name) { return getenv(name); }
#else
const char* lab_env(const char*) { return nullptr; }
#endif
void attention_lab_switches(AttnArgs& a) {
  static const int sw[2] = {
      (lab_env("RVB_ATTN_OCC") && atoi(lab_env("RVB_ATTN_OCC")) == 3 ? ATTN_LAB_OCC3 : 0) |
          (lab_env("RVB_ATTN_MF") && atoi(lab_env("RVB_ATTN_MF")) == 0 ? ATTN_LAB_MF1 : 0) |
          (lab_env("RVB_ATTN_PADK") && atoi(lab_env("RVB_ATTN_PADK")) == 16 ? ATTN_LAB_PADK16 : 0),
      lab_env("RVB_ATTN_PLAIN") ? atoi(lab_env("RVB_ATTN_PLAIN")) : 0};
  a.lab |= sw[0];
  if (sw[1]) a.plain_order = 1;
}
}
extern "C" {

int rvb_model_cfg_size(void) { return (int)sizeof(rvb_model_cfg); }

int rvb_wer_counts(const int32_t* ref, int64_t n_ref, const int32_t* hyp, int64_t n_hyp, int64_t* counts) {
  if ((!ref && n_ref > 0) || (!hyp && n_hyp > 0) || !counts || n_ref < 0 || n_hyp < 0) { set_error("rvb_wer_counts: bad argument"); return E_ARG; }
  edit_counts(ref, n_ref, hyp, n_hyp, counts);
  return OK;
}

int rvb_create(const rvb_model_cfg* cfg, int device, rvb_engine** out) {
  if (!cfg || !out) { set_error("rvb_create: null argument"); return E_ARG; }
  if (cfg->struct_size != (int32_t)sizeof(rvb_model_cfg)) {
    set_error("rvb_create: ABI mismatch: rvb_model_cfg.struct_size is " + std::to_string(cfg->struct_size) + ", this library's struct has " +
              std::to_string(sizeof(rvb_model_cfg)) + " bytes (bind it field by field from include/rvb.h)");
    return E_ARG;
  }
  if (cfg->dtype != RVB_F32 && cfg->dtype != RVB_BF16 && cfg->dtype != RVB_FP8) { set_error("rvb_create: bad dtype"); return E_ARG; }
  if (cfg->d_model <= 0 || cfg->heads <= 0 || cfg->d_model % cfg->heads || cfg->d_model % 8 || cfg->ffn_dim % 8 ||
      cfg->dec_ffn_dim % 8 || cfg->input_dim != 80 || cfg->vocab < 2 || cfg->num_blocks < 1 ||
      cfg->cnn_kernel < 1 || cfg->cnn_kernel > 31 || (!cfg->cnn_causal && (cfg->cnn_kernel % 2) == 0) ||
      cfg->chunk_frames < 7 || cfg->max_chunks < 1 ||
      (cfg->dec_blocks > 0 && (cfg->dec_heads <= 0 || cfg->d_model % cfg->dec_heads))) {
    set_error("rvb_create: unsupported model dimensions (need d, ffn dims % 8 == 0, d % heads == 0, input_dim 80, cnn kernel <= 31 and odd unless causal)");
    return E_ARG;
  }
  int ndev = 0;
  hipError_t err = hipGetDeviceCount(&ndev);
  if (err != hipSuccess || ndev <= 0) { set_error("no HIP device available: librvb has no CPU fallback"); return E_HIP; }
  if (device < 0 || device >= ndev) { set_error("rvb_create: device index out of range"); return E_ARG; }
  RVB_HIP_CHECK(hipSetDevice(device));
  rvb_engine* e = new rvb_engine();
  e->cfg = *cfg; e->device = device;
  e->fp8 = cfg->dtype == RVB_FP8;
  e->dtype = e->fp8 ? (int)DT_BF16 : cfg->dtype;
  hipError_t se = hipStreamCreateWithFlags(&e->stream, hipStreamNonBlocking);
  if (se != hipSuccess) { delete e; set_error("hipStreamCreate failed"); return E_HIP; }
  *out = e;
  return OK;
}

void rvb_destroy(rvb_engine* e) {
  if (!e) return;
  (void)rvb_comm_destroy(e);
  (void)hipSetDevice(e->device);
  (void)hipStreamSynchronize(e->stream);
  DevBuf* bufs[] = {&e->cmvn_mean, &e->cmvn_istd, &e->conv1_w, &e->conv1_b, &e->pe_f32, &e->stage, &e->pcm, &e->feats,
                    &e->d_feats_in, &e->X1, &e->X2, &e->x, &e->xn, &e->y, &e->h, &e->ao, &e->dconv, &e->enc_out,
                    &e->logits, &e->topv, &e->topi, &e->d_enc_lens, &e->d_seq_start, &e->d_seq_len, &e->d_aux_i32,
                    &e->dx, &e->dxn, &e->dy, &e->dh, &e->dqkv, &e->dq, &e->dao, &e->kvmem, &e->d_tok, &e->d_pos,
                    &e->d_tgt, &e->d_logp, &e->d_hq_start, &e->d_hq_len, &e->d_hkv_start, &e->d_hkv_len,
                    &e->d_hq_pos0, &e->d_hpath_start, &e->d_hpath_len, &e->d_path, &e->d_work, &e->d_tgt_ptr,
                    &e->fb_window, &e->fb_twiddle, &e->fb_melw, &e->fb_lo, &e->fb_hi,
                    &e->conv2.w, &e->conv2.b, &e->embed_out.w, &e->embed_out.b, &e->ctc.w, &e->ctc.b,
                    &e->enc_after.g, &e->enc_after.b};
  for (DevBuf* b : bufs) b->release();
  e->aligner.release();
  e->graph_aligner.release();
  e->finder.release();
  e->scorer.release();
  for (DevBuf* b : {&e->align_lp, &e->align_tv, &e->align_ti, &e->align_row, &e->align_col, &e->align_out}) b->release();
  e->d_xlse.release(); e->d_xsum.release(); e->d_xtop.release();
  e->atopv.release(); e->atopi.release(); e->d_stream_i32.release(); e->d_amax.release(); e->d_f8sat.release();
  e->wave_f32.release(); e->wave_in.release(); e->rs_kernel.release();
  e->jlogp.release(); e->jpair_row.release(); e->jpair_tok.release(); e->jpair_out.release();
  for (auto& b : e->jkv) b.release();
  for (auto* v : {&e->stream_st.kv, &e->stream_st.kv2, &e->stream_st.cnn, &e->stream_st.cnn2}) for (auto& b : *v) b.release();
  for (auto* v : {&e->kcache, &e->vcache, &e->kcache2, &e->vcache2, &e->memkv}) for (auto& b : *v) b.release();
  auto rel_lin = [](Linear& l) { l.w.release(); l.b.release(); l.w8.release(); l.wscale.release(); };
  auto rel_n = [](LNorm& n) { n.g.release(); n.b.release(); };
  for (auto& L : e->enc) {
    for (Linear* l : {&L.ffm1, &L.ffm2, &L.ff1, &L.ff2, &L.qkv, &L.att_out, &L.pw1, &L.pw1_glu, &L.pw2, &L.lsl}) rel_lin(*l);
    for (LNorm* n : {&L.n_ffm, &L.n_mha, &L.n_conv, &L.n_ff, &L.n_final, &L.n_cnn}) rel_n(*n);
    L.pos_keys.release(); L.pos_bias.release(); L.bias_u.release(); L.bias_v.release(); L.dw_w.release(); L.dw_b.release();
  }
  for (Decoder* D : {&e->dec_l, &e->dec_r}) {
    D->embed.release(); rel_lin(D->out); rel_n(D->after);
    for (auto& L : D->layers) {
      for (Linear* l : {&L.self_qkv, &L.self_out, &L.src_q, &L.src_kv, &L.src_out, &L.ff1, &L.ff2, &L.lsl}) rel_lin(*l);
      for (LNorm* n : {&L.n1, &L.n2, &L.n3}) rel_n(*n);
      L.kvmem.release();
    }
  }
  if (e->h_topv) (void)hipHostFree(e->h_topv);
  if (e->h_topi) (void)hipHostFree(e->h_topi);
  for (auto& sl : e->slices) if (!sl.done) (void)hipEventDestroy(sl.ev);
  for (auto ev : e->slice_event_pool) (void)hipEventDestroy(ev);
  for (auto& p : e->pending) { (void)hipEventDestroy(p.a); (void)hipEventDestroy(p.b); }
  for (auto ev : e->event_pool) (void)hipEventDestroy(ev);
  if (e->copy_stream) (void)hipStreamDestroy(e->copy_stream);
  if (e->pcm_ready) (void)hipEventDestroy(e->pcm_ready);
  if (e->pcm_free) (void)hipEventDestroy(e->pcm_free);
  e->pcm_next.release();
  (void)hipStreamDestroy(e->stream);
  delete e;
}

int rvb_load_tensor(rvb_engine* e, const char* name, const float* host, const int64_t* shape, int ndim) {
  if (!e || !name || !host || ndim < 0 || (ndim > 0 && !shape)) { set_error("rvb_load_tensor: null argument"); return E_ARG; }
  HostTensor t;
  size_t n = 1;
  for (int i = 0; i < ndim; ++i) { if (shape[i] < 0) { set_error("negative dim"); return E_ARG; } t.shape.push_back(shape[i]); n *= (size_t)shape[i]; }
  t.data.assign(host, host + n);
  e->host[name] = std::move(t);
  return OK;
}

int rvb_finalize(rvb_engine* e, const float* cat_embs, int n_cat) {
  if (!e || (n_cat > 0 && !cat_embs)) { set_error("rvb_finalize: null argument"); return E_ARG; }
  return finalize_impl(e, cat_embs, n_cat);
}

int64_t rvb_num_frames(int64_t n) { return n < 400 ? 0 : 1 + (n - 400) / 160; }

static int drop_pending_upload(rvb_engine* e) {
  if (e->pcm_pending) {
    RVB_HIP_CHECK(hipStreamSynchronize(e->copy_stream));
    e->pcm_pending = false;
  }
  return OK;
}

int rvb_upload_pcm(rvb_engine* e, const int16_t* pcm, int64_t n) {
  if (!e || (!pcm && n > 0) || n < 0) { set_error("rvb_upload_pcm: bad argument"); return E_ARG; }
  RVB_HIP_CHECK(hipSetDevice(e->device));
  RVB_TRY(drop_pending_upload(e));
  RVB_TRY(e->pcm.ensure((size_t)n * 2 + 16));
  if (n) RVB_HIP_CHECK(hipMemcpyAsync(e->pcm.p, pcm, (size_t)n * 2, hipMemcpyHostToDevice, e->stream));
  RVB_HIP_CHECK(hipStreamSynchronize(e->stream));
  e->n_samples = n;
  e->pcm_is_float = false;
  return OK;
}

int rvb_upload_pcm_async(rvb_engine* e, const int16_t* pcm, int64_t n) {
  if (!e || (!pcm && n > 0) || n < 0) { set_error("rvb_upload_pcm_async: bad argument"); return E_ARG; }
  if (e->pcm_pending) { set_error("rvb_upload_pcm_async: an upload is already pending (consumed by the next rvb_fbank)"); return E_STATE; }
  RVB_HIP_CHECK(hipSetDevice(e->device));
  if (!e->copy_stream) {
    RVB_HIP_CHECK(hipStreamCreateWithFlags(&e->copy_stream, hipStreamNonBlocking));
    RVB_HIP_CHECK(hipEventCreateWithFlags(&e->pcm_ready, hipEventDisableTiming));
    RVB_HIP_CHECK(hipEventCreateWithFlags(&e->pcm_free, hipEventDisableTiming));
  }
  else RVB_HIP_CHECK(hipStreamWaitEvent(e->copy_stream, e->pcm_free, 0));
  RVB_TRY(e->pcm_next.ensure((size_t)n * 2 + 16));
  if (n) RVB_HIP_CHECK(hipMemcpyAsync(e->pcm_next.p, pcm, (size_t)n * 2, hipMemcpyHostToDevice, e->copy_stream));
  RVB_HIP_CHECK(hipEventRecord(e->pcm_ready, e->copy_stream));
  e->n_samples_next = n;
  e->pcm_pending = true;
  return OK;
}

int rvb_host_alloc(void** out, int64_t bytes) {
  if (!out || bytes < 0) { set_error("rvb_host_alloc: bad argument"); return E_ARG; }
  *out = nullptr;
  hipError_t err = hipHostMalloc(out, (size_t)std::max<int64_t>(bytes, 16), hipHostMallocDefault);
  if (err != hipSuccess) { *out = nullptr; set_error(std::string("hipHostMalloc: ") + hipGetErrorString(err)); return E_NOMEM; }
  return OK;
}
int rvb_host_free(void* p) {
  if (p) RVB_HIP_CHECK(hipHostFree(p));
  return OK;
}

int rvb_set_fp8_policy(rvb_engine* e, int groups, int first_block, int last_block) {
  if (!e) { set_error("rvb_set_fp8_policy: null engine"); return E_ARG; }
  if (!e->fp8) { set_error("rvb_set_fp8_policy: not an RVB_FP8 engine"); return E_STATE; }
  if (groups > 63 || first_block < 0) { set_error("rvb_set_fp8_policy: groups is a 6-bit mask (bit 5: the subsampling's conv2), first_block >= 0"); return E_ARG; }
// ... 3 lines not shown
int rvb_set_decoding_chunk(rvb_engine* e, int chunk_size, int num_left_chunks) {
  if (!e) { set_error("rvb_set_decoding_chunk: null engine"); return E_ARG; }
  if (chunk_size > 4095 || num_left_chunks > 4094) { set_error("rvb_set_decoding_chunk: value too large"); return E_ARG; }
  e->dec_chunk = chunk_size > 0 ? chunk_size : 0;
  e->dec_left = num_left_chunks < 0 ? -1 : num_left_chunks;
  return OK;
}

static int resample_uploaded(rvb_engine* e, bool src_float, int64_t n, int sample_rate) {
  const int target = 16000;
  std::vector<float> ker;
  int orig, nw, width, K;
  resample_taps(sample_rate, target, &ker, &orig, &nw, &width, &K);
  const int64_t n_out = (nw * n + orig - 1) / orig;
  RVB_TRY(e->rs_kernel.ensure(ker.size() * 4));
  RVB_TRY(e->wave_f32.ensure((size_t)std::max<int64_t>(n_out, 1) * 4));
  RVB_HIP_CHECK(hipMemcpyAsync(e->rs_kernel.p, ker.data(), ker.size() * 4, hipMemcpyHostToDevice, e->stream));
  {
    Scope sc(e, "resample");
    if (src_float) RVB_TRY(resample_f32(e->stream, e->wave_in.as<float>(), n, e->rs_kernel.as<float>(), orig, nw, width, K, e->wave_f32.as<float>(), n_out));
    else RVB_TRY(resample(e->stream, e->pcm.as<int16_t>(), n, e->rs_kernel.as<float>(), orig, nw, width, K, e->wave_f32.as<float>(), n_out));
  }
  RVB_HIP_CHECK(hipStreamSynchronize(e->stream));
  e->n_samples = n_out;
  e->pcm_is_float = true;
  return OK;
}

int rvb_upload_pcm_rate(rvb_engine* e, const int16_t* pcm, int64_t n, int sample_rate) {
  if (sample_rate == 16000) return rvb_upload_pcm(e, pcm, n);
  if (!e || (!pcm && n > 0) || n < 0 || sample_rate < 1000 || sample_rate > 384000) { set_error("rvb_upload_pcm_rate: bad argument"); return E_ARG; }
  RVB_HIP_CHECK(hipSetDevice(e->device));
  RVB_TRY(drop_pending_upload(e));
  RVB_TRY(e->pcm.ensure((size_t)n * 2 + 16));
  if (n) RVB_HIP_CHECK(hipMemcpyAsync(e->pcm.p, pcm, (size_t)n * 2, hipMemcpyHostToDevice, e->stream));
  return resample_uploaded(e, false, n, sample_rate);
}

int rvb_upload_wave_f32(rvb_engine* e, const float* wave, int64_t n, int sample_rate) {
  if (!e || (!wave && n > 0) || n < 0 || sample_rate < 1000 || sample_rate > 384000) { set_error("rvb_upload_wave_f32: bad argument"); return E_ARG; }
  RVB_HIP_CHECK(hipSetDevice(e->device));
  RVB_TRY(drop_pending_upload(e));
  rvb::DevBuf& dst = sample_rate == 16000 ? e->wave_f32 : e->wave_in;
  RVB_TRY(dst.ensure((size_t)std::max<int64_t>(n, 1) * 4));
  if (n) RVB_HIP_CHECK(hipMemcpyAsync(dst.p, wave, (size_t)n * 4, hipMemcpyHostToDevice, e->stream));
  if (sample_rate != 16000) return resample_uploaded(e, true, n, sample_rate);
  RVB_HIP_CHECK(hipStreamSynchronize(e->stream));
  e->n_samples = n;
  e->pcm_is_float = true;
  return OK;
}

int rvb_get_waveform(rvb_engine* e, float* out, int64_t* n) {
  if (!e) { set_error("rvb_get_waveform: null engine"); return E_ARG; }
  RVB_HIP_CHECK(hipSetDevice(e->device));
  if (n) *n = e->n_samples;
  if (!out || e->n_samples == 0) return OK;
  if (e->pcm_is_float) {
    RVB_HIP_CHECK(hipMemcpy(out, e->wave_f32.p, (size_t)e->n_samples * 4, hipMemcpyDeviceToHost));
  } else {
    std::vector<int16_t> tmp(e->n_samples);
    RVB_HIP_CHECK(hipMemcpy(tmp.data(), e->pcm.p, (size_t)e->n_samples * 2, hipMemcpyDeviceToHost));
    for (int64_t i = 0; i < e->n_samples; ++i) out[i] = (float)tmp[i];
  }
  return OK;
}

int rvb_fbank(rvb_engine* e, float* feats_out, int64_t* n_frames) {
  if (!e) { set_error("rvb_fbank: null engine"); return E_ARG; }
  if (!e->fb_window.p) { set_error("rvb_fbank before rvb_finalize"); return E_STATE; }
  RVB_HIP_CHECK(hipSetDevice(e->device));
  if (e->pcm_pending) {
    RVB_HIP_CHECK(hipStreamWaitEvent(e->stream, e->pcm_ready, 0));
    std::swap(e->pcm, e->pcm_next);
    e->n_samples = e->n_samples_next;
    e->pcm_is_float = false;
    e->pcm_pending = false;
  }
  const int64_t nf = rvb_num_frames(e->n_samples);
  const int64_t T0 = e->cfg.chunk_frames;
  const int64_t rows = nf + T0;
  RVB_TRY(e->feats.ensure((size_t)std::max<int64_t>(rows, 1) * 80 * 4));
  RVB_HIP_CHECK(hipMemsetAsync((char*)e->feats.p + (size_t)nf * 80 * 4, 0, (size_t)std::max<int64_t>(rows - nf, 1) * 80 * 4, e->stream));
  FbankTables t{e->fb_window.as<float>(), e->fb_twiddle.as<float>(), e->fb_melw.as<float>(), e->fb_lo.as<int>(), e->fb_hi.as<int>()};
  {
    Scope sc(e, "fbank");
    if (e->pcm_is_float) RVB_TRY(fbank_f32(e->stream, e->wave_f32.as<float>(), nf, e->feats.as<float>(), t));
    else RVB_TRY(fbank(e->stream, e->pcm.as<int16_t>(), nf, e->feats.as<float>(), t));
  }
  if (e->copy_stream) RVB_HIP_CHECK(hipEventRecord(e->pcm_free, e->stream));
  if (feats_out && nf) {
    RVB_HIP_CHECK(hipMemcpyAsync(feats_out, e->feats.p, (size_t)nf * 80 * 4, hipMemcpyDeviceToHost, e->stream));
    RVB_HIP_CHECK(hipStreamSynchronize(e->stream));
  }
  e->n_frames = nf; e->feat_rows = rows;
  if (n_frames) *n_frames = nf;
  return OK;
}

int rvb_encode(rvb_engine* e, const float* feats, int64_t first_chunk, const int32_t* lens, int B, int T0, int beam,
               float blank_penalty) {
  if (!e || !lens) { set_error("rvb_encode: null argument"); return E_ARG; }
  return encode_impl(e, feats, first_chunk, lens, B, T0, beam, blank_penalty);
}

int rvb_stream_begin(rvb_engine* e) {
  if (!e) { set_error("rvb_stream_begin: null engine"); return E_ARG; }
  return stream_begin_impl(e);
}
int rvb_stream_chunk(rvb_engine* e, const float* feats, int n_frames, int required_cache_size, float* out, int32_t* n_out) {
  if (!e || !feats) { set_error("rvb_stream_chunk: null argument"); return E_ARG; }
  return stream_chunk_impl(e, feats, n_frames, required_cache_size, out, n_out);
}
int rvb_stream_state(rvb_engine* e, int32_t* offset, int32_t* cache_frames) {
  if (!e) { set_error("rvb_stream_state: null engine"); return E_ARG; }
  if (offset) *offset = e->stream_st.offset;
  if (cache_frames) *cache_frames = e->stream_st.cache_len;
  return OK;
}
int rvb_stream_finish(rvb_engine* e, int beam, float blank_penalty) {
  if (!e) { set_error("rvb_stream_finish: null engine"); return E_ARG; }
  return stream_finish_impl(e, beam, blank_penalty);
}

int rvb_encoder_frames(rvb_engine* e, int32_t* T_out) {
  if (!e || !T_out || e->B <= 0) { set_error("no encoded batch"); return E_STATE; }
  *T_out = e->T2; return OK;
}
int rvb_get_encoder_lens(rvb_engine* e, int32_t* lens) {
  if (!e || !lens || e->B <= 0) { set_error("no encoded batch"); return E_STATE; }
  memcpy(lens, e->enc_lens.data(), (size_t)e->B * 4); return OK;
}
int rvb_get_encoder_out(rvb_engine* e, float* out) {
  if (!e || !out || e->B <= 0) { set_error("no encoded batch"); return E_STATE; }
  const size_t n = (size_t)e->B * e->T2 * e->cfg.d_model;
  RVB_HIP_CHECK(hipSetDevice(e->device));
  RVB_TRY(wait_slices(e, -1));
  RVB_HIP_CHECK(hipStreamSynchronize(e->stream));
  if (e->dtype == DT_F32) {
    RVB_HIP_CHECK(hipMemcpy(out, e->enc_out.p, n * 4, hipMemcpyDeviceToHost));
  } else {
    std::vector<bf16_t> tmp(n);
    RVB_HIP_CHECK(hipMemcpy(tmp.data(), e->enc_out.p, n * 2, hipMemcpyDeviceToHost));
    for (size_t i = 0; i < n; ++i) out[i] = bf16_to_f32(tmp[i]);
  }
  return OK;
}
int rvb_get_ctc_logprobs(rvb_engine* e, int chunk, float* out) {
  if (!e || !out || e->B <= 0 || chunk < 0 || chunk >= e->B) { set_error("rvb_get_ctc_logprobs: bad chunk"); return E_ARG; }
  RVB_HIP_CHECK(hipSetDevice(e->device));
  const int d = e->cfg.d_model, V = e->cfg.vocab, T = e->T2, Vld = (V + 3) & ~3;
  if (T > LOGIT_SLAB) { set_error("chunk too long for the logit slab"); return E_UNSUPPORTED; }
  RVB_TRY(wait_slices(e, -1));
  DevBuf lp, tv, ti;
  RVB_TRY(lp.ensure((size_t)T * V * 4)); RVB_TRY(tv.ensure((size_t)T * 4)); RVB_TRY(ti.ensure((size_t)T * 4));
  int r = run_gemm(e, (const char*)e->enc_out.p + (size_t)chunk * T * d * dt_size(e->dtype), d, e->ctc, e->logits.p, Vld, T, true);
  if (r == OK) r = logsoftmax_topk(e->stream, e->logits.as<float>(), T, V, Vld, 1, 0.f, e->cfg.blank_id, tv.as<float>(), ti.as<int>(), lp.as<float>());
  if (r == OK && hipMemcpyAsync(out, lp.p, (size_t)T * V * 4, hipMemcpyDeviceToHost, e->stream) != hipSuccess) r = E_HIP;
  (void)hipStreamSynchronize(e->stream);
  lp.release(); tv.release(); ti.release();
  return r;
}
int rvb_get_ctc_topk(rvb_engine* e, float* vals, int32_t* idx) {
  if (!e || e->B <= 0) { set_error("no encoded batch"); return E_STATE; }
  const size_t n = (size_t)e->B * e->T2 * e->beam;
  RVB_TRY(wait_slices(e, -1));
  if (vals) memcpy(vals, e->h_topv, n * 4);
// ... 654 lines not shown
  return OK;
}

}

#ifdef RVB_TEST_API
#include "test_api.h"
extern "C" int rvb_test_build_trie(const int32_t* tokens, const int32_t* lens, const int32_t* chunk_of, int n_hyps, int n_chunks, int sos,
                                   int eos, int reversed, int32_t* n_rows, int32_t* tok, int32_t* pos, int32_t* path, int32_t* hq_start,
                                   int32_t* hq_len, int32_t* hq_pos0, int32_t* tgt_ptr, int32_t* tgt, int32_t* pair_slot, int32_t* n_work) {
  if (!tokens || !lens || !chunk_of || !n_rows || n_hyps < 0) { set_error("rvb_test_build_trie: bad argument"); return E_ARG; }
  std::vector<HypRef> hyps;
  std::vector<int> first(n_hyps);
  int P = 0, off = 0;
  for (int i = 0; i < n_hyps; ++i) { hyps.push_back({chunk_of[i], i, lens[i], P}); first[i] = off; P += lens[i] + 1; off += lens[i]; }
  TrieBatch t;
  auto seq = [&](const HypRef& h, int j) { return tokens[first[h.idx] + (reversed ? h.len - 1 - j : j)]; };
  build_trie_range(hyps.data(), hyps.data() + hyps.size(), 0, n_chunks, sos, eos, seq, &t);
  {
    std::vector<TrieBatch> part(std::max(n_chunks, 0));
    size_t a = 0;
    for (int b = 0; b < n_chunks; ++b) {
      size_t z = a;
      while (z < hyps.size() && hyps[z].chunk == b) ++z;
      build_trie_range(hyps.data() + a, hyps.data() + z, b, 1, sos, eos, seq, &part[b]);
      a = z;
    }
    TrieBatch m;
    merge_tries(part, &m);
    const bool same = m.R == t.R && m.P == t.P && m.max_chunk_rows == t.max_chunk_rows && m.tok == t.tok && m.pos == t.pos &&
                      m.path == t.path && m.hq_start == t.hq_start && m.hq_len == t.hq_len && m.hq_pos0 == t.hq_pos0 &&
                      m.hkv_start == t.hkv_start && m.hkv_len == t.hkv_len && m.crow_start == t.crow_start &&
                      m.crow_len == t.crow_len && m.tgt_ptr == t.tgt_ptr && m.tgt == t.tgt && m.pair_slot == t.pair_slot &&
                      m.work == t.work;
    if (a != hyps.size() || !same) {
      std::string which;
#define RVB_DIFF(f) if (!(m.f == t.f)) which += std::string(" ") + #f;
      RVB_DIFF(R) RVB_DIFF(P) RVB_DIFF(max_chunk_rows) RVB_DIFF(tok) RVB_DIFF(pos) RVB_DIFF(path) RVB_DIFF(hq_start) RVB_DIFF(hq_len)
      RVB_DIFF(hq_pos0) RVB_DIFF(hkv_start) RVB_DIFF(hkv_len) RVB_DIFF(crow_start) RVB_DIFF(crow_len) RVB_DIFF(tgt_ptr) RVB_DIFF(tgt)
      RVB_DIFF(pair_slot) RVB_DIFF(work)
#undef RVB_DIFF
      set_error("rvb_test_build_trie: the stitched per-chunk tries differ from the batch trie in:" + which);
      return E_STATE;
    }
  }
  *n_rows = t.R;
  if (n_work) *n_work = (int32_t)t.work.size() / 2;
  auto cp = [](int32_t* dst, const std::vector<int32_t>& v) { if (dst) memcpy(dst, v.data(), v.size() * 4); };
  cp(tok, t.tok); cp(pos, t.pos); cp(path, t.path); cp(hq_start, t.hq_start); cp(hq_len, t.hq_len); cp(hq_pos0, t.hq_pos0);
  cp(tgt_ptr, t.tgt_ptr); cp(tgt, t.tgt); cp(pair_slot, t.pair_slot);
  return OK;
}

extern "C" int rvb_test_host_pool(int n_threads, int items, int rounds) {
  if (n_threads < 1 || items < 0 || rounds < 1) { set_error("rvb_test_host_pool: bad argument"); return E_ARG; }
  HostPool pool;
  std::vector<std::atomic<int>> hits(items);
  for (int r = 0; r < rounds; ++r) {
    for (auto& h : hits) h.store(0);
    std::atomic<int> next(0), entered(0);
    const unsigned n = (unsigned)std::max(1, n_threads - (r % 3));
    pool.run(n, [&] {
      entered.fetch_add(1);
      for (int i = next.fetch_add(1); i < items; i = next.fetch_add(1)) hits[i].fetch_add(1);
    });
    if (entered.load() != (int)n) { set_error("rvb_test_host_pool: a job was not run by the requested number of threads"); return E_STATE; }
    for (int i = 0; i < items; ++i)
      if (hits[i].load() != 1) { set_error("rvb_test_host_pool: work item executed " + std::to_string(hits[i].load()) + " times"); return E_STATE; }
  }
  return OK;
}

extern "C" int rvb_test_fbank(const int16_t* pcm, int64_t n_samples, float* feats) {
  int ndev = 0;
  if (hipGetDeviceCount(&ndev) != hipSuccess || ndev <= 0) { set_error("no HIP device available: librvb has no CPU fallback"); return E_HIP; }
  if (!pcm || !feats) { set_error("rvb_test_fbank: null argument"); return E_ARG; }
  rvb_engine e;
  RVB_TRY(make_fbank_tables(&e));
  const int64_t nf = rvb_num_frames(n_samples);
  DevBuf dp, df;
  RVB_TRY(dp.ensure((size_t)n_samples * 2 + 16));
  RVB_TRY(df.ensure((size_t)std::max<int64_t>(nf, 1) * 80 * 4));
  RVB_HIP_CHECK(hipMemcpy(dp.p, pcm, (size_t)n_samples * 2, hipMemcpyHostToDevice));
  FbankTables t{e.fb_window.as<float>(), e.fb_twiddle.as<float>(), e.fb_melw.as<float>(), e.fb_lo.as<int>(), e.fb_hi.as<int>()};
  int r = fbank(nullptr, dp.as<int16_t>(), nf, df.as<float>(), t);
  if (r == OK && hipDeviceSynchronize() != hipSuccess) { set_error("fbank kernel failed"); r = E_HIP; }
  if (r == OK && nf && hipMemcpy(feats, df.p, (size_t)nf * 80 * 4, hipMemcpyDeviceToHost) != hipSuccess) r = E_HIP;
  dp.release(); df.release();
  for (DevBuf* b : {&e.fb_window, &e.fb_twiddle, &e.fb_melw, &e.fb_lo, &e.fb_hi}) b->release();
  return r;
}
#endif
```

### reverb_amd/csrc/fbank.hip

```cpp
#include <algorithm>
#include <cmath>
#include <vector>

#include "../../include/rvb.h"
#include "common.h"
#include "kernels.h"

namespace rvb {

static constexpr int WIN = 400, SHIFT = 160, NFFT = 512, NBIN = 257, NMEL = 80;

template <typename In>
__global__ __launch_bounds__(256) void fbank_kernel(const In* __restrict__ pcm, int64_t n_frames,
                                                    float* __restrict__ feats, FbankTables t) {
  __shared__ float s_re[4][NFFT];
  __shared__ float s_im[4][NFFT];
  const int lane = threadIdx.x & 63;
  const int w = threadIdx.x >> 6;
  const int64_t frame = (int64_t)blockIdx.x * 4 + w;
  const bool live = frame < n_frames;
  float* re = s_re[w];
  float* im = s_im[w];

  float x[7];
  float sum = 0.f;
  const In* src = pcm + frame * SHIFT;
#pragma unroll
  for (int i = 0; i < 7; ++i) {
    const int j = lane + 64 * i;
    x[i] = (live && j < WIN) ? (float)src[j] : 0.f;
    sum += x[i];
  }
  const float mean = wave_sum(sum) / (float)WIN;
#pragma unroll
  for (int i = 0; i < 7; ++i) {
    const int j = lane + 64 * i;
    if (j < WIN) im[j] = x[i] - mean;
  }
  __syncthreads();
  float y[8];
#pragma unroll
  for (int i = 0; i < 8; ++i) {
    const int j = lane + 64 * i;
    float v = 0.f;
    if (j < WIN) {
      const float cur = im[j];
      const float prev = im[j > 0 ? j - 1 : 0];
      v = (cur - 0.97f * prev) * t.window[j];
    }
    y[i] = v;
  }
  __syncthreads();
#pragma unroll
  for (int i = 0; i < 8; ++i) {
    const int j = lane + 64 * i;
    re[__brev((unsigned)j) >> 23] = y[i];
    im[j] = 0.f;
  }
  __syncthreads();
#pragma unroll 1
  for (int s = 0; s < 9; ++s) {
    const int half = 1 << s;
#pragma unroll
    for (int q = 0; q < 4; ++q) {
      const int b = lane + 64 * q;
      const int j = b & (half - 1);
      const int i0 = ((b >> s) << (s + 1)) + j;
      const int i1 = i0 + half;
      const int tw = j << (8 - s);
      const float wr = t.twiddle[2 * tw], wi = t.twiddle[2 * tw + 1];
      const float ar = re[i0], ai = im[i0], br = re[i1], bi = im[i1];
      const float tr = wr * br - wi * bi;
      const float ti = wr * bi + wi * br;
      re[i0] = ar + tr; im[i0] = ai + ti;
      re[i1] = ar - tr; im[i1] = ai - ti;
    }
    __syncthreads();
  }
  float pw[5];
#pragma unroll
  for (int i = 0; i < 5; ++i) {
    const int j = lane + 64 * i;
    pw[i] = (j < NBIN) ? re[j] * re[j] + im[j] * im[j] : 0.f;
  }
  __syncthreads();
#pragma unroll
  for (int i = 0; i < 5; ++i) {
    const int j = lane + 64 * i;
    if (j < NBIN) re[j] = pw[i];
  }
  __syncthreads();
  if (live) {
#pragma unroll
    for (int i = 0; i < 2; ++i) {
      const int m = lane + 64 * i;
      if (m < NMEL) {
        const int lo = t.mel_lo[m], hi = t.mel_hi[m];
        const float* wrow = t.mel_w + (size_t)m * NBIN;
        float acc = 0.f;
        for (int b = lo; b < hi; ++b) acc += re[b] * wrow[b];
        feats[frame * NMEL + m] = logf(fmaxf(acc, 1.1920928955078125e-07f));
      }
    }
  }
}

int fbank(hipStream_t s, const int16_t* pcm, int64_t n_frames, float* feats, const FbankTables& t) {
  if (n_frames <= 0) return OK;
  hipLaunchKernelGGL(fbank_kernel<int16_t>, dim3(cdiv(n_frames, 4)), dim3(256), 0, s, pcm, n_frames, feats, t);
  RVB_HIP_CHECK(hipGetLastError());
  return OK;
}

int fbank_f32(hipStream_t s, const float* wave, int64_t n_frames, float* feats, const FbankTables& t) {
  if (n_frames <= 0) return OK;
  hipLaunchKernelGGL(fbank_kernel<float>, dim3(cdiv(n_frames, 4)), dim3(256), 0, s, wave, n_frames, feats, t);
  RVB_HIP_CHECK(hipGetLastError());
  return OK;
}

template <typename In>
__global__ __launch_bounds__(256) void resample_kernel(const In* __restrict__ pcm, int64_t n_in, const float* __restrict__ ker,
                                                       int orig, int new_, int width, int K, float* __restrict__ out,
                                                       int64_t n_out) {
  const int64_t n = (int64_t)blockIdx.x * 256 + threadIdx.x;
  if (n >= n_out) return;
  const int64_t j = n / new_;
  const int p = (int)(n - j * new_);
  const int64_t base = j * orig - width;
  const float* kr = ker + (size_t)p * K;
  float acc = 0.f;
  for (int k = 0; k < K; ++k) {
    const int64_t i = base + k;
    if (i >= 0 && i < n_in) acc = fmaf(kr[k], (float)pcm[i], acc);
  }
  out[n] = acc;
}
int resample(hipStream_t s, const int16_t* pcm, int64_t n_in, const float* ker, int orig, int new_, int width, int K, float* out,
             int64_t n_out) {
  if (n_out <= 0) return OK;
  hipLaunchKernelGGL(resample_kernel<int16_t>, dim3(cdiv(n_out, 256)), dim3(256), 0, s, pcm, n_in, ker, orig, new_, width, K, out, n_out);
  RVB_HIP_CHECK(hipGetLastError());
  return OK;
}

int resample_f32(hipStream_t s, const float* pcm, int64_t n_in, const float* ker, int orig, int new_, int width, int K, float* out,
             int64_t n_out) {
  if (n_out <= 0) return OK;
  hipLaunchKernelGGL(resample_kernel<float>, dim3(cdiv(n_out, 256)), dim3(256), 0, s, pcm, n_in, ker, orig, new_, width, K, out, n_out);
  RVB_HIP_CHECK(hipGetLastError());
  return OK;
}

void resample_taps(int sample_rate, int target, std::vector<float>* ker, int* orig_out, int* new_out, int* width_out, int* K_out) {
  int a = sample_rate, b = target;
  while (b) { const int t = a % b; a = b; b = t; }
  const int orig = sample_rate / a, nw = target / a;
  const double lpw = 6.0, rolloff = 0.99;
  const double base_freq = std::min(orig, nw) * rolloff;
  const int width = (int)std::ceil(lpw * orig / base_freq);
  const int K = 2 * width + orig;
  ker->assign((size_t)nw * K, 0.f);
  const double PI = 3.14159265358979323846;
  for (int p = 0; p < nw; ++p)
    for (int k = 0; k < K; ++k) {
      double t = (-(double)p / nw + (double)(k - width) / orig) * base_freq;
      t = std::max(-lpw, std::min(lpw, t));
      const double c = std::cos(t * PI / lpw / 2.0);
      const double window = c * c;
      t *= PI;
      const double sinc = t == 0.0 ? 1.0 : std::sin(t) / t;
      (*ker)[(size_t)p * K + k] = (float)(sinc * window * (base_freq / orig));
    }
  *orig_out = orig; *new_out = nw; *width_out = width; *K_out = K;
}

struct FbankAny { int win, shift, nmel; };
__global__ __launch_bounds__(256) void fbank_any_kernel(const float* __restrict__ wave, int64_t n_frames, float* __restrict__ feats,
                                                        FbankTables t, FbankAny g) {
  __shared__ float s_re[4][NFFT];
  __shared__ float s_im[4][NFFT];
  const int lane = threadIdx.x & 63;
  const int w = threadIdx.x >> 6;
  const int64_t frame = (int64_t)blockIdx.x * 4 + w;
  const bool live = frame < n_frames;
  float* re = s_re[w];
  float* im = s_im[w];
  float x[8];
  float sum = 0.f;
  const float* src = wave + frame * g.shift;
#pragma unroll
  for (int i = 0; i < 8; ++i) {
    const int j = lane + 64 * i;
    x[i] = (live && j < g.win) ? src[j] : 0.f;
    sum += x[i];
  }
  const float mean = wave_sum(sum) / (float)g.win;
#pragma unroll
  for (int i = 0; i < 8; ++i) {
    const int j = lane + 64 * i;
// ... 147 lines not shown
```

### reverb_amd/csrc/kernels.h

```cpp
#pragma once
#include <vector>
#include "common.h"

namespace rvb {

enum { DT_F32 = 0, DT_BF16 = 1 };
enum { ACT_NONE = 0, ACT_SILU = 1, ACT_RELU = 2, ACT_LRELU = 3  };
enum { ACT_GLU = 4 };

inline size_t dt_size(int dt) { return dt == DT_BF16 ? 2 : 4; }

struct GemmArgs {
  const void* A;
  const void* W;
  const float* bias;
  const float* res;
  void* C;
  int M, N, K;
  int lda, ldw, ldc, ldres;
  float alpha;
  int act;
  int out_f32;
  int conv;
  int cT1, cF1, cT2, cF2, cC;
  int group_m, prio;
  int res_epilogue;
  int fast_epilogue;
  int stagger_ticks, stagger_first;
  int k_serp;
  int in_fp8, out_fp8;
  float a_scale, out_inv_scale;
  const float* w_scale;
  unsigned* sat;
  long long* dbg;
  const void* rowadd;
  int rowadd_rows, rowadd_ld, rowadd_col0, rowadd_cols;
};
int gemm(hipStream_t s, int dtype, const GemmArgs& a);
bool gemm2_applicable(int dtype, const GemmArgs& a);
bool gemm_glu_supported(int dtype, const GemmArgs& a);
int gemm2(hipStream_t s, int dtype, const GemmArgs& a);
extern int g_gemm_variant;
extern int g_gemm2_flags, g_gemm2_group_m;

struct FbankTables {
  const float* window;
  const float* twiddle;
  const float* mel_w;
  const int* mel_lo;
  const int* mel_hi;
};
int fbank(hipStream_t s, const int16_t* pcm, int64_t n_frames, float* feats, const FbankTables& t);
int fbank_f32(hipStream_t s, const float* wave, int64_t n_frames, float* feats, const FbankTables& t);
void resample_taps(int sample_rate, int target, std::vector<float>* ker, int* orig, int* new_, int* width, int* K);
int round_to_i16(hipStream_t s, const float* x, int64_t n, int16_t* out);
int resample(hipStream_t s, const int16_t* pcm, int64_t n_in, const float* ker, int orig, int new_, int width, int K, float* out,
             int64_t n_out);
int resample_f32(hipStream_t s, const float* wave, int64_t n_in, const float* ker, int orig, int new_, int width, int K, float* out,
             int64_t n_out);

int subsample_conv1(hipStream_t s, int dtype, const float* feats, const float* mean, const float* istd,
                    const float* w , const float* b , void* out, int B, int T0, int F0,
                    int d, float out_fp8_scale = 0.f , unsigned* amax = nullptr ,
                    unsigned* sat = nullptr );

enum { NORM_LN = 0, NORM_AFFINE = 1 };
struct NormArgs {
  const float* x;
  int x_bf16 = 0;
  const float* gamma;
  const float* beta;
  float eps;
  int mode;
  int silu;
  const void* add;
  void* out;
  int out_f32;
  int M, d;
  const float* gamma2 = nullptr;
  const float* beta2 = nullptr;
  float eps2 = 0.f;
  void* out2 = nullptr;
  int out_fp8 = 0, out2_fp8 = 0;
  float out_inv_scale = 1.f, out2_inv_scale = 1.f;
  unsigned* sat = nullptr;
  unsigned* sat2 = nullptr;
};
int rownorm(hipStream_t s, int dtype, const NormArgs& a);

struct GluDwArgs {
  const void* G;
  const float* pw1_bias;
  const float* dw_w;
  const float* dw_b;
  const int* lens;
  float* out;
  int B, T, d, K;
  int out_bf16 = 0;
  int gated = 0;
  int causal = 0;
  const void* hist = nullptr;
  int hist_rows = 0;
};
int glu_dwconv(hipStream_t s, int dtype, const GluDwArgs& a);

int embed_tokens(hipStream_t s, const float* E, const float* pe, const int* tok, const int* pos, float* out,
                 int rows, int d, float scale);

int logsoftmax_topk(hipStream_t s, const float* logits, int M, int V, int ld, int k, float blank_penalty,
                    int blank_id, float* topk_val, int* topk_idx, float* logp_out);

int lse_gather(hipStream_t s, const float* logits, int R, int V, int ld, const int* target, float* out, float blank_penalty = 0.f,
               int blank_id = -1);
int lse_gather_multi(hipStream_t s, const float* logits, int R, int V, int ld, const int* ptr, const int* target, float* out);
int row_xent(hipStream_t s, const float* logits, int R, int V, int ld, const int* ptr, const int* target, float* logp, float* lse,
             double* sum_x, int* top1);

int gather_pairs(hipStream_t s, const float* table, size_t ld, const int* row, const int* col, int n, float* out);

int gather_cache(hipStream_t s, const void* src, void* dst, const int* parent, int R, int L, int rows, int row_bytes);

int amax_abs(hipStream_t s, int dtype, const void* x, size_t n, float* slot);

int convert_f32(hipStream_t s, int dtype, const float* src, void* dst, size_t n);

enum { CTC_ALIGN_MAX_TOKENS = 16383,
       CTC_ALIGN_MAX_STATES = 2 * CTC_ALIGN_MAX_TOKENS + 1,
       CTC_ALIGN_MAX_FRAMES = 1 << 20 };
struct VitSeq {
  int L, S, T;
  int tok_off;
  int frame_off;
  int f0, f1;
  int pad_;
// ... 199 lines not shown
```

Baseline: 27860.

## Pack decoder trie uploads into one pinned transfer and rewrite fbank kernel

The decoder forward pass previously made thirteen separate int32 uploads per rescoring batch. It now packs them into one pinned host buffer and sends them with a single async copy, addressing each array by offset, which cuts per-call transfer and launch overhead. Separately, the fbank kernel is rewritten as a register radix-8 FFT with wavefront-only syncs. It handles several frames per wave, caches the window, twiddle and compacted mel weights in LDS, and uses a compact mel weight table. The fbank rewrite adds a new table requirement and a cap on mel weights, and could change numerics slightly.

```diff
diff --git a/reverb_amd/_lib.py b/reverb_amd/_lib.py
--- a/reverb_amd/_lib.py
+++ b/reverb_amd/_lib.py
@@ -210,6 +210,7 @@
     "rvb_test_build_trie": (C.c_int, [_i32p, _i32p, _i32p, C.c_int, C.c_int, C.c_int, C.c_int, C.c_int, _i32p, _i32p, _i32p, _i32p, _i32p, _i32p,
                                       _i32p, _i32p, _i32p, _i32p, _i32p]),
     "rvb_test_fbank": (C.c_int, [_i16p, C.c_int64, _f32p]),
+    "rvb_test_fbank_forms": (C.c_int, [C.c_int, C.c_int, C.c_void_p, C.c_int64, _f32p]),
     "rvb_test_set_gemm_variant": (C.c_int, [C.c_int]),
     "rvb_test_set_gemm2_opts": (C.c_int, [C.c_int, C.c_int]),
     "rvb_test_gemm_timeline": (C.c_int, [C.c_int] * 6 + [C.POINTER(C.c_longlong), C.c_int, _i32p]),
diff --git a/reverb_amd/csrc/diar_engine.hip b/reverb_amd/csrc/diar_engine.hip
--- a/reverb_amd/csrc/diar_engine.hip
+++ b/reverb_amd/csrc/diar_engine.hip
@@ -57,7 +57,7 @@
   DevBuf stem_w, stem_b;
   std::vector<std::vector<ResBlock>> stages;
   Linear seg1;
-  DevBuf fb_window, fb_twiddle, fb_melw, fb_lo, fb_hi;
+  DevBuf fb_window, fb_twiddle, fb_melw, fb_lo, fb_hi, fb_melcw, fb_meloff;
   DevBuf pcm_pad, emb_fb;
   int64_t emb_frames = 0;
   int nfr = 0;
@@ -361,7 +361,12 @@
   RVD_TRY(up_f32(e, e->fb_twiddle, tw.data(), tw.size()));
   RVD_TRY(up_f32(e, e->fb_melw, melw.data(), melw.size()));
   RVD_TRY(up_f32(e, e->fb_lo, (const float*)lo.data(), lo.size()));
-  return up_f32(e, e->fb_hi, (const float*)hi.data(), hi.size());
+  RVD_TRY(up_f32(e, e->fb_hi, (const float*)hi.data(), hi.size()));
+  std::vector<float> cw;
+  std::vector<int32_t> off;
+  RVD_TRY(fbank_compact_mel(melw, lo, hi, &cw, &off));
+  RVD_TRY(up_f32(e, e->fb_melcw, cw.data(), cw.size()));
+  return up_f32(e, e->fb_meloff, (const float*)off.data(), off.size());
 }
 
 int pack_conv_bn(rvd_engine* e, ConvW& c, const std::string& conv, const std::string& bn, int cout, int cin, int k, int stride) {
@@ -789,7 +794,7 @@
   for (auto& n : e->norm) { n.g.release(); n.b.release(); }
   for (auto& l : e->lstm) { l.ih.w.release(); l.ih.b.release(); l.whh.release(); }
   for (auto& l : e->lin) { l.w.release(); l.b.release(); }
-  DevBuf* ebufs[] = {&e->stem_w, &e->stem_b, &e->seg1.w, &e->seg1.b, &e->fb_window, &e->fb_twiddle, &e->fb_melw, &e->fb_lo, &e->fb_hi,
+  DevBuf* ebufs[] = {&e->stem_w, &e->stem_b, &e->seg1.w, &e->seg1.b, &e->fb_window, &e->fb_twiddle, &e->fb_melw, &e->fb_lo, &e->fb_hi, &e->fb_melcw, &e->fb_meloff,
                      &e->pcm_pad, &e->emb_fb, &e->e_win, &e->e_mean, &e->e_item_b, &e->e_mask, &e->e_stats, &e->e_out};
   for (auto* b : ebufs) b->release();
   for (auto& st : e->stages)
@@ -893,7 +898,8 @@
     RVB_HIP_CHECK(hipMemsetAsync(e->pcm_pad.p, 0, (size_t)e->n_pad * 2, e->stream));
     RVB_HIP_CHECK(hipMemcpyAsync(e->pcm_pad.p, e->pcm.p, (size_t)n * 2, hipMemcpyDeviceToDevice, e->stream));
     DScope sc(e, "emb_fbank");
-    FbankTables t{e->fb_window.as<float>(), e->fb_twiddle.as<float>(), e->fb_melw.as<float>(), e->fb_lo.as<int>(), e->fb_hi.as<int>()};
+    FbankTables t{e->fb_window.as<float>(), e->fb_twiddle.as<float>(), e->fb_melw.as<float>(), e->fb_lo.as<int>(), e->fb_hi.as<int>(),
+                  e->fb_melcw.as<float>(), e->fb_meloff.as<int>()};
     RVD_TRY(fbank(e->stream, e->pcm_pad.as<int16_t>(), e->emb_frames, e->emb_fb.as<float>(), t));
     RVD_TRY(e->e_mean.ensure((size_t)e->n_windows * FB_MEL * 4));
     RVD_TRY(emb_window_mean(e->stream, e->emb_fb.as<float>(), nullptr, (int)e->n_windows, c.step_samples / FB_SHIFT, e->nfr, e->e_mean.as<float>()));
diff --git a/reverb_amd/csrc/engine.h b/reverb_amd/csrc/engine.h
--- a/reverb_amd/csrc/engine.h
+++ b/reverb_amd/csrc/engine.h
@@ -226,7 +226,7 @@
   rvb::Decoder dec_l, dec_r;
   rvb::DevBuf pe_f32;
   int pe_rows = 0;
-  rvb::DevBuf fb_window, fb_twiddle, fb_melw, fb_lo, fb_hi;
+  rvb::DevBuf fb_window, fb_twiddle, fb_melw, fb_lo, fb_hi, fb_melcw, fb_meloff;
   rvb::DevBuf stage;
 
   rvb::DevBuf pcm, feats;
@@ -269,7 +269,10 @@
   std::vector<rvb::DevBuf> kcache, vcache, kcache2, vcache2, memkv;
   rvb::DevBuf dx, dxn, dy, dh, dqkv, dq, dao, kvmem, d_tok, d_pos, d_tgt, d_logp;
   rvb::DevBuf d_hq_start, d_hq_len, d_hkv_start, d_hkv_len;
-  rvb::DevBuf d_hq_pos0, d_hpath_start, d_hpath_len, d_path, d_work, d_tgt_ptr;
+  rvb::DevBuf d_hpath_start, d_hpath_len, d_path;
+  void* h_trie = nullptr;
+  size_t h_trie_cap = 0;
+  rvb::DevBuf d_trie;
   int64_t rescore_rows = 0, rescore_pairs = 0;
   rvb::DevBuf d_xlse, d_xsum, d_xtop;
 
diff --git a/reverb_amd/csrc/engine.hip b/reverb_amd/csrc/engine.hip
--- a/reverb_amd/csrc/engine.hip
+++ b/reverb_amd/csrc/engine.hip
@@ -1,4 +1,5 @@
 #include "engine.h"
+#include "stage_pack.h"
 
 #include <algorithm>
 #include <atomic>
@@ -209,6 +210,11 @@
   RVB_TRY(upload_f32(e, e->fb_melw, melw.data(), melw.size()));
   RVB_TRY(upload_i32(e, e->fb_lo, lo.data(), lo.size()));
   RVB_TRY(upload_i32(e, e->fb_hi, hi.data(), hi.size()));
+  std::vector<float> cw;
+  std::vector<int32_t> off;
+  RVB_TRY(fbank_compact_mel(melw, lo, hi, &cw, &off));
+  RVB_TRY(upload_f32(e, e->fb_melcw, cw.data(), cw.size()));
+  RVB_TRY(upload_i32(e, e->fb_meloff, off.data(), off.size()));
   RVB_HIP_CHECK(hipStreamSynchronize(e->stream));
   return OK;
 }
@@ -1122,25 +1128,41 @@
   return OK;
 }
 
+static int trie_stage_reserve(rvb_engine* e, size_t bytes) {
+  const size_t cap = pack_grow(e->h_trie_cap, bytes);
+  if (cap == e->h_trie_cap && e->h_trie) return OK;
+  if (e->h_trie) { (void)hipHostFree(e->h_trie); e->h_trie = nullptr; e->h_trie_cap = 0; }
+  hipError_t err = hipHostMalloc(&e->h_trie, cap, hipHostMallocDefault);
+  if (err != hipSuccess) {
+    e->h_trie = nullptr;
+    (void)hipGetLastError();
+    set_error("hipHostMalloc of " + std::to_string(cap) + " bytes failed: " + hipGetErrorString(err));
+    return E_NOMEM;
+  }
+  e->h_trie_cap = cap;
+  return OK;
+}
+
 struct XentRows { std::vector<float> lse; std::vector<double> sum_x; std::vector<int32_t> top1; };
 static int decoder_forward(rvb_engine* e, Decoder& D, const TrieBatch& t, std::vector<float>* logp, XentRows* xent = nullptr) {
   const rvb_model_cfg& c = e->cfg;
   const int d = c.d_model, heads = c.dec_heads, dk = d / heads, ff = c.dec_ffn_dim, V = c.vocab;
   const int M = e->B * e->T2, R = t.R, nhyp = (int)t.hq_start.size();
   const size_t es = dt_size(e->dtype);
-  RVB_TRY(upload_i32(e, e->d_tok, t.tok.data(), R));
-  RVB_TRY(upload_i32(e, e->d_pos, t.pos.data(), R));
-  RVB_TRY(upload_i32(e, e->d_tgt, t.tgt.data(), t.P));
-  RVB_TRY(upload_i32(e, e->d_tgt_ptr, t.tgt_ptr.data(), R + 1));
-  RVB_TRY(upload_i32(e, e->d_path, t.path.data(), t.path.size()));
-  RVB_TRY(upload_i32(e, e->d_work, t.work.data(), t.work.size()));
-  RVB_TRY(upload_i32(e, e->d_hq_start, t.hq_start.data(), nhyp));
-  RVB_TRY(upload_i32(e, e->d_hq_len, t.hq_len.data(), nhyp));
-  RVB_TRY(upload_i32(e, e->d_hq_pos0, t.hq_pos0.data(), nhyp));
-  RVB_TRY(upload_i32(e, e->d_hpath_start, t.hkv_start.data(), nhyp));
-  RVB_TRY(upload_i32(e, e->d_hpath_len, t.hkv_len.data(), nhyp));
-  RVB_TRY(upload_i32(e, e->d_hkv_start, t.crow_start.data(), e->B));
-  RVB_TRY(upload_i32(e, e->d_hkv_len, t.crow_len.data(), e->B));
+  enum { I_TOK, I_POS, I_TGT, I_TGT_PTR, I_PATH, I_WORK, I_HQ_START, I_HQ_LEN, I_HQ_POS0, I_HPATH_START, I_HPATH_LEN, I_CROW_START,
+         I_CROW_LEN, I_COUNT };
+  const PackItem items[I_COUNT] = {
+      {t.tok.data(), (size_t)R}, {t.pos.data(), (size_t)R}, {t.tgt.data(), (size_t)t.P}, {t.tgt_ptr.data(), (size_t)R + 1},
+      {t.path.data(), t.path.size()}, {t.work.data(), t.work.size()}, {t.hq_start.data(), (size_t)nhyp},
+      {t.hq_len.data(), (size_t)nhyp}, {t.hq_pos0.data(), (size_t)nhyp}, {t.hkv_start.data(), (size_t)nhyp},
+      {t.hkv_len.data(), (size_t)nhyp}, {t.crow_start.data(), (size_t)e->B}, {t.crow_len.data(), (size_t)e->B}};
+  size_t off[I_COUNT];
+  const size_t trie_bytes = pack_offsets(items, I_COUNT, off);
+  RVB_TRY(trie_stage_reserve(e, trie_bytes));
+  pack_copy(e->h_trie, trie_bytes, items, I_COUNT, off);
+  RVB_TRY(e->d_trie.ensure(trie_bytes));
+  RVB_HIP_CHECK(hipMemcpyAsync(e->d_trie.p, e->h_trie, trie_bytes, hipMemcpyHostToDevice, e->stream));
+  auto dev = [&](int i) { return (const int*)((const char*)e->d_trie.p + off[i]); };
   RVB_TRY(e->dx.ensure((size_t)R * d * 4));
   RVB_TRY(e->dxn.ensure((size_t)R * d * es));
   RVB_TRY(e->dy.ensure((size_t)R * d * es));
@@ -1156,7 +1178,7 @@
   float* x = e->dx.as<float>();
   {
     Scope sc(e, "embed");
-    RVB_TRY(embed_tokens(e->stream, D.embed.as<float>(), e->pe_f32.as<float>(), e->d_tok.as<int>(), e->d_pos.as<int>(),
+    RVB_TRY(embed_tokens(e->stream, D.embed.as<float>(), e->pe_f32.as<float>(), dev(I_TOK), dev(I_POS),
                          x, R, d, std::sqrt((float)d)));
   }
   for (auto& L : D.layers) {
@@ -1166,9 +1188,9 @@
     memset(&a, 0, sizeof(a));
     a.q = e->dqkv.p; a.k = (const char*)e->dqkv.p + (size_t)d * es; a.v = (const char*)e->dqkv.p + (size_t)2 * d * es;
     a.q_stride = a.k_stride = a.v_stride = 3 * d; a.o_stride = d; a.out = e->dao.p;
-    a.q_start = e->d_hq_start.as<int>(); a.q_len = e->d_hq_len.as<int>(); a.q_pos0 = e->d_hq_pos0.as<int>();
-    a.kv_start = e->d_hpath_start.as<int>(); a.kv_len = e->d_hpath_len.as<int>(); a.kv_index = e->d_path.as<int>();
-    a.work = e->d_work.as<int>(); a.n_work = (int)t.work.size() / 2; a.q_block = 16;
+    a.q_start = dev(I_HQ_START); a.q_len = dev(I_HQ_LEN); a.q_pos0 = dev(I_HQ_POS0);
+    a.kv_start = dev(I_HPATH_START); a.kv_len = dev(I_HPATH_LEN); a.kv_index = dev(I_PATH);
+    a.work = dev(I_WORK); a.n_work = (int)t.work.size() / 2; a.q_block = 16;
     a.nseq = nhyp; a.heads = heads; a.dk = dk; a.max_q = 16; a.causal = 1; a.sqrt_dk = std::sqrt((float)dk);
     {
       Scope sc(e, "attention");
@@ -1180,7 +1202,7 @@
     memset(&a, 0, sizeof(a));
     a.q = e->dq.p; a.k = L.kvmem.p; a.v = (const char*)L.kvmem.p + (size_t)d * es;
     a.q_stride = d; a.k_stride = a.v_stride = 2 * d; a.o_stride = d; a.out = e->dao.p;
-    a.q_start = e->d_hkv_start.as<int>(); a.q_len = e->d_hkv_len.as<int>();
+    a.q_start = dev(I_CROW_START); a.q_len = dev(I_CROW_LEN);
     a.kv_start = e->d_aux_i32.as<int>(); a.kv_len = e->d_aux_i32.as<int>() + e->B;
     a.nseq = e->B; a.heads = heads; a.dk = dk; a.max_q = t.max_chunk_rows; a.causal = 0; a.sqrt_dk = std::sqrt((float)dk);
     {
@@ -1204,10 +1226,10 @@
     RVB_TRY(run_gemm(e, (const char*)e->dxn.p + (size_t)r0 * d * es, d, D.out, e->logits.p, Vld, rows, true));
     Scope sc(e, "lse_gather");
     if (xent)
-      RVB_TRY(row_xent(e->stream, e->logits.as<float>(), rows, V, Vld, e->d_tgt_ptr.as<int>() + r0, e->d_tgt.as<int>(),
+      RVB_TRY(row_xent(e->stream, e->logits.as<float>(), rows, V, Vld, dev(I_TGT_PTR) + r0, dev(I_TGT),
                        e->d_logp.as<float>(), e->d_xlse.as<float>() + r0, e->d_xsum.as<double>() + r0, e->d_xtop.as<int>() + r0));
     else
-      RVB_TRY(lse_gather_multi(e->stream, e->logits.as<float>(), rows, V, Vld, e->d_tgt_ptr.as<int>() + r0, e->d_tgt.as<int>(),
+      RVB_TRY(lse_gather_multi(e->stream, e->logits.as<float>(), rows, V, Vld, dev(I_TGT_PTR) + r0, dev(I_TGT),
                                e->d_logp.as<float>()));
   }
   logp->resize(t.P);
@@ -1832,8 +1854,8 @@
                     &e->logits, &e->topv, &e->topi, &e->d_enc_lens, &e->d_seq_start, &e->d_seq_len, &e->d_aux_i32,
                     &e->dx, &e->dxn, &e->dy, &e->dh, &e->dqkv, &e->dq, &e->dao, &e->kvmem, &e->d_tok, &e->d_pos,
                     &e->d_tgt, &e->d_logp, &e->d_hq_start, &e->d_hq_len, &e->d_hkv_start, &e->d_hkv_len,
-                    &e->d_hq_pos0, &e->d_hpath_start, &e->d_hpath_len, &e->d_path, &e->d_work, &e->d_tgt_ptr,
-                    &e->fb_window, &e->fb_twiddle, &e->fb_melw, &e->fb_lo, &e->fb_hi,
+                    &e->d_hpath_start, &e->d_hpath_len, &e->d_path,
+                    &e->fb_window, &e->fb_twiddle, &e->fb_melw, &e->fb_lo, &e->fb_hi, &e->fb_melcw, &e->fb_meloff,
                     &e->conv2.w, &e->conv2.b, &e->embed_out.w, &e->embed_out.b, &e->ctc.w, &e->ctc.b,
                     &e->enc_after.g, &e->enc_after.b};
   for (DevBuf* b : bufs) b->release();
@@ -1866,6 +1888,8 @@
   }
   if (e->h_topv) (void)hipHostFree(e->h_topv);
   if (e->h_topi) (void)hipHostFree(e->h_topi);
+  if (e->h_trie) (void)hipHostFree(e->h_trie);
+  e->d_trie.release();
   for (auto& sl : e->slices) if (!sl.done) (void)hipEventDestroy(sl.ev);
   for (auto ev : e->slice_event_pool) (void)hipEventDestroy(ev);
   for (auto& p : e->pending) { (void)hipEventDestroy(p.a); (void)hipEventDestroy(p.b); }
@@ -2035,7 +2059,8 @@
   const int64_t rows = nf + T0;
   RVB_TRY(e->feats.ensure((size_t)std::max<int64_t>(rows, 1) * 80 * 4));
   RVB_HIP_CHECK(hipMemsetAsync((char*)e->feats.p + (size_t)nf * 80 * 4, 0, (size_t)std::max<int64_t>(rows - nf, 1) * 80 * 4, e->stream));
-  FbankTables t{e->fb_window.as<float>(), e->fb_twiddle.as<float>(), e->fb_melw.as<float>(), e->fb_lo.as<int>(), e->fb_hi.as<int>()};
+  FbankTables t{e->fb_window.as<float>(), e->fb_twiddle.as<float>(), e->fb_melw.as<float>(), e->fb_lo.as<int>(), e->fb_hi.as<int>(),
+                e->fb_melcw.as<float>(), e->fb_meloff.as<int>()};
   {
     Scope sc(e, "fbank");
     if (e->pcm_is_float) RVB_TRY(fbank_f32(e->stream, e->wave_f32.as<float>(), nf, e->feats.as<float>(), t));
@@ -2856,12 +2881,12 @@
   RVB_TRY(dp.ensure((size_t)n_samples * 2 + 16));
   RVB_TRY(df.ensure((size_t)std::max<int64_t>(nf, 1) * 80 * 4));
   RVB_HIP_CHECK(hipMemcpy(dp.p, pcm, (size_t)n_samples * 2, hipMemcpyHostToDevice));
-  FbankTables t{e.fb_window.as<float>(), e.fb_twiddle.as<float>(), e.fb_melw.as<float>(), e.fb_lo.as<int>(), e.fb_hi.as<int>()};
+  FbankTables t{e.fb_window.as<float>(), e.fb_twiddle.as<float>(), e.fb_melw.as<float>(), e.fb_lo.as<int>(), e.fb_hi.as<int>(), e.fb_melcw.as<float>(), e.fb_meloff.as<int>()};
   int r = fbank(nullptr, dp.as<int16_t>(), nf, df.as<float>(), t);
   if (r == OK && hipDeviceSynchronize() != hipSuccess) { set_error("fbank kernel failed"); r = E_HIP; }
   if (r == OK && nf && hipMemcpy(feats, df.p, (size_t)nf * 80 * 4, hipMemcpyDeviceToHost) != hipSuccess) r = E_HIP;
   dp.release(); df.release();
-  for (DevBuf* b : {&e.fb_window, &e.fb_twiddle, &e.fb_melw, &e.fb_lo, &e.fb_hi}) b->release();
+  for (DevBuf* b : {&e.fb_window, &e.fb_twiddle, &e.fb_melw, &e.fb_lo, &e.fb_hi, &e.fb_melcw, &e.fb_meloff}) b->release();
   return r;
 }
 #endif
diff --git a/reverb_amd/csrc/fbank.hip b/reverb_amd/csrc/fbank.hip
--- a/reverb_amd/csrc/fbank.hip
+++ b/reverb_amd/csrc/fbank.hip
@@ -1,5 +1,6 @@
 #include <algorithm>
 #include <cmath>
+#include <string>
 #include <vector>
 
 #include "../../include/rvb.h"
@@ -9,113 +10,163 @@
 namespace rvb {
 
 static constexpr int WIN = 400, SHIFT = 160, NFFT = 512, NBIN = 257, NMEL = 80;
+static constexpr int MEL_CW_MAX = 512;
+
+static constexpr int FPW = 4, FPB = 4 * FPW;
+static constexpr int XP = NFFT + 64;
+static constexpr int PWP = 260;
+
+__device__ inline void wave_lds_sync() {
+  __builtin_amdgcn_fence(__ATOMIC_RELEASE, "wavefront");
+  __builtin_amdgcn_wave_barrier();
+  __builtin_amdgcn_fence(__ATOMIC_ACQUIRE, "wavefront");
+}
+
+template <int K>
+__device__ inline void fft_phase(float (&re)[8], float (&im)[8], int lowp, const float2* tw) {
+#pragma clang fp contract(off)
+#pragma unroll
+  for (int t = 0; t < 3; ++t) {
+    const int s = 3 * K + t;
+#pragma unroll
+    for (int q = 0; q < 4; ++q) {
+      const int r0 = ((q >> t) << (t + 1)) | (q & ((1 << t) - 1));
+      const int r1 = r0 | (1 << t);
+      const int j = ((r0 & ((1 << t) - 1)) << (3 * K)) + lowp;
+      const float2 wv = tw[j << (8 - s)];
+      const float wr = wv.x, wi = wv.y;
+      const float ar = re[r0], ai = im[r0], br = re[r1], bi = im[r1];
+      const float tr = __builtin_fmaf(wr, br, -(wi * bi));
+      const float ti = __builtin_fmaf(wi, br, wr * bi);
+      re[r0] = ar + tr; im[r0] = ai + ti;
+      re[r1] = ar - tr; im[r1] = ai - ti;
+    }
+  }
+}
 
 template <typename In>
-__global__ __launch_bounds__(256) void fbank_kernel(const In* __restrict__ pcm, int64_t n_frames,
-                                                    float* __restrict__ feats, FbankTables t) {
-  __shared__ float s_re[4][NFFT];
-  __shared__ float s_im[4][NFFT];
-  const int lane = threadIdx.x & 63;
-  const int w = threadIdx.x >> 6;
-  const int64_t frame = (int64_t)blockIdx.x * 4 + w;
-  const bool live = frame < n_frames;
-  float* re = s_re[w];
-  float* im = s_im[w];
-
-  float x[7];
-  float sum = 0.f;
-  const In* src = pcm + frame * SHIFT;
-#pragma unroll
-  for (int i = 0; i < 7; ++i) {
-    const int j = lane + 64 * i;
-    x[i] = (live && j < WIN) ? (float)src[j] : 0.f;
-    sum += x[i];
-  }
-  const float mean = wave_sum(sum) / (float)WIN;
-#pragma unroll
-  for (int i = 0; i < 7; ++i) {
-    const int j = lane + 64 * i;
-    if (j < WIN) im[j] = x[i] - mean;
-  }
-  __syncthreads();
-  float y[8];
-#pragma unroll
-  for (int i = 0; i < 8; ++i) {
-    const int j = lane + 64 * i;
-    float v = 0.f;
-    if (j < WIN) {
-      const float cur = im[j];
-      const float prev = im[j > 0 ? j - 1 : 0];
-      v = (cur - 0.97f * prev) * t.window[j];
-    }
-    y[i] = v;
-  }
-  __syncthreads();
-#pragma unroll
-  for (int i = 0; i < 8; ++i) {
-    const int j = lane + 64 * i;
-    re[__brev((unsigned)j) >> 23] = y[i];
-    im[j] = 0.f;
-  }
-  __syncthreads();
+__global__ __launch_bounds__(256) void fbank_kernel(const In* __restrict__ pcm, int64_t n_frames, float* __restrict__ feats,
+                                                    FbankTables t) {
+#pragma clang fp contract(off)
+  __shared__ float s_win[WIN];
+  __shared__ float2 s_tw[NFFT / 2];
+  __shared__ float s_mw[MEL_CW_MAX];
+  __shared__ int s_mlo[NMEL], s_moff[NMEL + 1];
+  __shared__ float s_re[4][XP];
+  __shared__ float s_im[4][XP];
+  __shared__ float s_pw[4][FPW][PWP];
+  const int tid = threadIdx.x, lane = tid & 63, w = tid >> 6;
+  for (int i = tid; i < WIN; i += 256) s_win[i] = t.window[i];
+  s_tw[tid] = make_float2(t.twiddle[2 * tid], t.twiddle[2 * tid + 1]);
+  const int n_cw = min(t.mel_off[NMEL], MEL_CW_MAX);
+  for (int i = tid; i < n_cw; i += 256) s_mw[i] = t.mel_cw[i];
+  if (tid < NMEL) s_mlo[tid] = t.mel_lo[tid];
+  if (tid <= NMEL) s_moff[tid] = t.mel_off[tid];
+  __syncthreads();
+
+  float* xr = s_re[w];
+  float* xi = s_im[w];
+  const int64_t frame0 = (int64_t)blockIdx.x * FPB + w;
+  const int rl = (int)(__brev((unsigned)lane) >> 26);
+  const int hi3 = lane >> 3, lo3 = lane & 7;
 #pragma unroll 1
-  for (int s = 0; s < 9; ++s) {
-    const int half = 1 << s;
-#pragma unroll
-    for (int q = 0; q < 4; ++q) {
-      const int b = lane + 64 * q;
-      const int j = b & (half - 1);
-      const int i0 = ((b >> s) << (s + 1)) + j;
-      const int i1 = i0 + half;
-      const int tw = j << (8 - s);
-      const float wr = t.twiddle[2 * tw], wi = t.twiddle[2 * tw + 1];
-      const float ar = re[i0], ai = im[i0], br = re[i1], bi = im[i1];
-      const float tr = wr * br - wi * bi;
-      const float ti = wr * bi + wi * br;
-      re[i0] = ar + tr; im[i0] = ai + ti;
-      re[i1] = ar - tr; im[i1] = ai - ti;
-    }
-    __syncthreads();
-  }
-  float pw[5];
-#pragma unroll
-  for (int i = 0; i < 5; ++i) {
-    const int j = lane + 64 * i;
-    pw[i] = (j < NBIN) ? re[j] * re[j] + im[j] * im[j] : 0.f;
-  }
-  __syncthreads();
-#pragma unroll
-  for (int i = 0; i < 5; ++i) {
-    const int j = lane + 64 * i;
-    if (j < NBIN) re[j] = pw[i];
-  }
-  __syncthreads();
-  if (live) {
-#pragma unroll
-    for (int i = 0; i < 2; ++i) {
-      const int m = lane + 64 * i;
-      if (m < NMEL) {
-        const int lo = t.mel_lo[m], hi = t.mel_hi[m];
-        const float* wrow = t.mel_w + (size_t)m * NBIN;
-        float acc = 0.f;
-        for (int b = lo; b < hi; ++b) acc += re[b] * wrow[b];
-        feats[frame * NMEL + m] = logf(fmaxf(acc, 1.1920928955078125e-07f));
+  for (int f = 0; f < FPW; ++f) {
+    const int64_t frame = frame0 + 4 * f;
+    if (frame >= n_frames) break;
+    float x[7];
+    float sum = 0.f;
+    const In* src = pcm + frame * SHIFT;
+#pragma unroll
+    for (int i = 0; i < 7; ++i) {
+      const int j = lane + 64 * i;
+      x[i] = (j < WIN) ? (float)src[j] : 0.f;
+      sum += x[i];
+    }
+    const float mean = wave_sum(sum) / (float)WIN;
+#pragma unroll
+    for (int i = 0; i < 7; ++i) {
+      const int j = lane + 64 * i;
+      if (j < WIN) xr[j] = x[i] - mean;
+    }
+    wave_lds_sync();
+    float re[8], im[8];
+#pragma unroll
+    for (int r = 0; r < 8; ++r) {
+      const int j = rl + 64 * (((r & 1) << 2) | (r & 2) | (r >> 2));
+      float v = 0.f;
+      if (j < WIN) {
+        const float cur = xr[j];
+        const float prev = xr[j > 0 ? j - 1 : 0];
+        v = __builtin_fmaf(-0.97f, prev, cur) * s_win[j];
       }
-    }
-  }
+      re[r] = v; im[r] = 0.f;
+    }
+    wave_lds_sync();
+    fft_phase<0>(re, im, 0, s_tw);
+#pragma unroll
+    for (int r = 0; r < 8; ++r) { xr[9 * lane + r] = re[r]; xi[9 * lane + r] = im[r]; }
+    wave_lds_sync();
+#pragma unroll
+    for (int r = 0; r < 8; ++r) { re[r] = xr[hi3 * 72 + r * 9 + lo3]; im[r] = xi[hi3 * 72 + r * 9 + lo3]; }
+    wave_lds_sync();
+    fft_phase<1>(re, im, lo3, s_tw);
+#pragma unroll
+    for (int r = 0; r < 8; ++r) { xr[hi3 * 72 + r * 8 + lo3] = re[r]; xi[hi3 * 72 + r * 8 + lo3] = im[r]; }
+    wave_lds_sync();
+#pragma unroll
+    for (int r = 0; r < 8; ++r) { re[r] = xr[r * 72 + lane]; im[r] = xi[r * 72 + lane]; }
+    wave_lds_sync();
+    fft_phase<2>(re, im, lane, s_tw);
+    float* pw = s_pw[w][f];
+#pragma unroll
+    for (int r = 0; r < 4; ++r) pw[lane + 64 * r] = __builtin_fmaf(re[r], re[r], im[r] * im[r]);
+    if (lane == 0) pw[256] = __builtin_fmaf(re[4], re[4], im[4] * im[4]);
+  }
+  wave_lds_sync();
+#pragma unroll 1
+  for (int task = lane; task < FPW * NMEL; task += 64) {
+    const int f = task / NMEL, m = task - f * NMEL;
+    const int64_t frame = frame0 + 4 * f;
+    if (frame >= n_frames) continue;
+    const float* pw = s_pw[w][f] + s_mlo[m];
+    const int o0 = s_moff[m], n = s_moff[m + 1] - o0;
+    const float* wrow = s_mw + o0;
+    float acc = 0.f;
+    for (int b = 0; b < n; ++b) acc = __builtin_fmaf(pw[b], wrow[b], acc);
+    feats[frame * NMEL + m] = logf(fmaxf(acc, 1.1920928955078125e-07f));
+  }
+}
+
+static int check_tables(const FbankTables& t) {
+  if (!t.mel_cw || !t.mel_off) { set_error("fbank: tables lack the compact mel weights (fbank_compact_mel)"); return E_ARG; }
+  return OK;
 }
 
 int fbank(hipStream_t s, const int16_t* pcm, int64_t n_frames, float* feats, const FbankTables& t) {
   if (n_frames <= 0) return OK;
-  hipLaunchKernelGGL(fbank_kernel<int16_t>, dim3(cdiv(n_frames, 4)), dim3(256), 0, s, pcm, n_frames, feats, t);
+  if (int r = check_tables(t)) return r;
+  hipLaunchKernelGGL(fbank_kernel<int16_t>, dim3(cdiv(n_frames, FPB)), dim3(256), 0, s, pcm, n_frames, feats, t);
   RVB_HIP_CHECK(hipGetLastError());
   return OK;
 }
 
 int fbank_f32(hipStream_t s, const float* wave, int64_t n_frames, float* feats, const FbankTables& t) {
   if (n_frames <= 0) return OK;
-  hipLaunchKernelGGL(fbank_kernel<float>, dim3(cdiv(n_frames, 4)), dim3(256), 0, s, wave, n_frames, feats, t);
-  RVB_HIP_CHECK(hipGetLastError());
+  if (int r = check_tables(t)) return r;
+  hipLaunchKernelGGL(fbank_kernel<float>, dim3(cdiv(n_frames, FPB)), dim3(256), 0, s, wave, n_frames, feats, t);
+  RVB_HIP_CHECK(hipGetLastError());
+  return OK;
+}
+
+int fbank_compact_mel(const std::vector<float>& melw, const std::vector<int32_t>& lo, const std::vector<int32_t>& hi,
+                      std::vector<float>* cw, std::vector<int32_t>* off) {
+  const int nmel = (int)lo.size();
+  cw->clear(); off->assign(1, 0);
+  for (int m = 0; m < nmel; ++m) {
+    for (int b = lo[m]; b < hi[m]; ++b) cw->push_back(melw[(size_t)m * NBIN + b]);
+    off->push_back((int32_t)cw->size());
+  }
+  if ((int)cw->size() > MEL_CW_MAX) { set_error("fbank: the mel triangles hold more than " + std::to_string(MEL_CW_MAX) + " weights"); return E_UNSUPPORTED; }
   return OK;
 }
 
diff --git a/reverb_amd/csrc/kernels.h b/reverb_amd/csrc/kernels.h
--- a/reverb_amd/csrc/kernels.h
+++ b/reverb_amd/csrc/kernels.h
@@ -49,7 +49,13 @@
   const float* mel_w;
   const int* mel_lo;
   const int* mel_hi;
-};
+  const float* mel_cw;
+  const int* mel_off;
+};
+int fbank_compact_mel(const std::vector<float>& melw, const std::vector<int32_t>& lo, const std::vector<int32_t>& hi,
+                      std::vector<float>* cw, std::vector<int32_t>* off);
+void fbank_host_tables(int win, int nmel, std::vector<float>* window, std::vector<float>* tw, std::vector<float>* melw,
+                       std::vector<int32_t>* lo, std::vector<int32_t>* hi);
 int fbank(hipStream_t s, const int16_t* pcm, int64_t n_frames, float* feats, const FbankTables& t);
 int fbank_f32(hipStream_t s, const float* wave, int64_t n_frames, float* feats, const FbankTables& t);
 void resample_taps(int sample_rate, int target, std::vector<float>* ker, int* orig, int* new_, int* width, int* K);
diff --git a/reverb_amd/csrc/stage_pack.h b/reverb_amd/csrc/stage_pack.h
--- /dev/null
+++ b/reverb_amd/csrc/stage_pack.h
@@ -0,0 +1,35 @@
+#pragma once
+#include <cstddef>
+#include <cstdint>
+#include <cstring>
+
+namespace rvb {
+
+struct PackItem { const int32_t* src; size_t n; };
+
+static constexpr size_t PACK_ALIGN = 16;
+inline size_t pack_slot_bytes(size_t n) { return (n * 4 + 16 + PACK_ALIGN - 1) & ~(PACK_ALIGN - 1); }
+
+inline size_t pack_offsets(const PackItem* items, int count, size_t* off) {
+  size_t at = 0;
+  for (int i = 0; i < count; ++i) { off[i] = at; at += pack_slot_bytes(items[i].n); }
+  return at;
+}
+
+inline size_t pack_grow(size_t cap, size_t need) {
+  if (need <= cap) return cap;
+  size_t c = cap ? cap : 4096;
+  while (c < need) c *= 2;
+  return c;
+}
+
+inline void pack_copy(void* block, size_t block_bytes, const PackItem* items, int count, const size_t* off) {
+  char* dst = (char*)block;
+  for (int i = 0; i < count; ++i) {
+    const size_t used = items[i].n * 4, end = (i + 1 < count) ? off[i + 1] : block_bytes;
+    if (used) memcpy(dst + off[i], items[i].src, used);
+    memset(dst + off[i] + used, 0, end - off[i] - used);
+  }
+}
+
+}
```

Result: no change. 28040, median of 6 (+0.6%).
